# yz-cnsdqz/PSI-release

Measured on AMD Instinct MI355X. Metric: fitting iters/sec (SMPL-X+SDF+Chamfer), PROX-E batch=32, higher is better.
Workload: dtype f32

## Files before the change

### include/psi_hip.h

```cpp
#ifndef PSI_HIP_H
#define PSI_HIP_H

#include <stdint.h>

#ifdef __cplusplus
extern "C" {
#endif

#define PSI_EINVAL (-22)
#define PSI_ETIMEOUT (-110)
#define PSI_ENOMEM (-12)

const char *psi_last_error(void);
int psi_version(void);
int psi_device_info(int *cu_count, int *wave_size, int *clock_khz, int *is_gfx950);

int psi_chamfer_arith_mode(void);
size_t psi_chamfer_workspace_bytes(int B, int n, int m);
int psi_chamfer_forward(const float *xyz1, const float *xyz2, int B, int n, int m,
                        float *dist1, int32_t *idx1, float *dist2, int32_t *idx2,
                        void *workspace, void *stream);
int psi_scratch_release(void *stream, int all);
int psi_chamfer_backward(const float *xyz1, const float *xyz2, float *gradxyz1, float *gradxyz2,
                         const float *graddist1, const float *graddist2,
                         const int32_t *idx1, const int32_t *idx2, int B, int n, int m, void *stream);

typedef struct psi_nn_index psi_nn_index;
int psi_nn_index_create(psi_nn_index **out, const float *h_points, int m);
void psi_nn_index_destroy(psi_nn_index *index);
int psi_nn_index_query(const psi_nn_index *index, const float *xyz1, int B, int n, float *dist1, int32_t *idx1,
                       int32_t *hint, void *stream);

typedef struct psi_nn_index_set psi_nn_index_set;
int psi_nn_index_set_create(psi_nn_index_set **out, const psi_nn_index *const *indices, int S);
void psi_nn_index_set_destroy(psi_nn_index_set *set);
int psi_nn_index_set_query(const psi_nn_index_set *set, const int32_t *slot, const float *xyz1, int B, int n,
                           float *dist1, int32_t *idx1, void *stream);

int psi_sdf_sample_forward(const float *sdf, const int32_t *scene_id, const float *gmin, const float *gmax,
                           const float *verts, int B, int V, int D, int S, int align_corners,
                           float *out_sdf, float *out_grad, void *stream);
int psi_sdf_sample_backward(const float *grad_sdf, const float *out_grad, int B, int V,
                            float *grad_verts, void *stream);
int psi_sdf_penetration_stats(const float *sdf_vals, long n, float *stats, void *stream);

typedef struct psi_lbs_model psi_lbs_model;
int psi_lbs_create(psi_lbs_model **out, const float *h_v_template, const float *h_shapedirs,
                   const float *h_posedirs, const float *h_J_regressor, const float *h_weights,
                   const int32_t *h_parents, int V, int J, int NB);
void psi_lbs_destroy(psi_lbs_model *model);
size_t psi_lbs_workspace_floats(const psi_lbs_model *model, int B);
int psi_lbs_forward(const psi_lbs_model *model, const float *betas, const float *pose, const float *transl,
                    const float *cam_ext, int B, float *verts, float *joints, float *ws, void *stream);
int psi_lbs_backward(const psi_lbs_model *model, const float *grad_verts, const float *betas, const float *pose,
                     const float *cam_ext, int B, float *ws, float *grad_betas, float *grad_pose,
                     float *grad_transl, void *stream);

typedef struct psi_fit_engine psi_fit_engine;
typedef struct psi_fit_config {
    int B, n_contact, m_scene, D, align_corners, world_size, num_pca_comps, max_history;
    int nn_mode;
    float w_rec, w_vposer, w_contact, w_collision, contact_const;
    float lr, beta1, beta2, eps;
    int independent_bodies;
    int concurrent_engines;
    double lr_d, beta1_d, beta2_d;
} psi_fit_config;
int psi_fit_create(psi_fit_engine **out, const psi_lbs_model *lbs, const psi_fit_config *cfg,
                   const float *h_w1, const float *h_b1, const float *h_w2, const float *h_b2,
                   const float *h_w3, const float *h_b3, const float *h_lh_comp, const float *h_rh_comp,
                   const float *h_pose_mean, const int32_t *h_contact_ids,
                   const float *d_scene_verts, const float *d_sdf, const float *h_gmin, const float *h_gmax);
void psi_fit_destroy(psi_fit_engine *engine);
typedef struct psi_fit_scene {
    const float *d_verts;
    const float *d_sdf;
    int m, D;
    float gmin[3], gmax[3];
} psi_fit_scene;
int psi_fit_create_scenes(psi_fit_engine **out, const psi_lbs_model *lbs, const psi_fit_config *cfg,
                          const float *h_w1, const float *h_b1, const float *h_w2, const float *h_b2,
                          const float *h_w3, const float *h_b3, const float *h_lh_comp, const float *h_rh_comp,
                          const float *h_pose_mean, const int32_t *h_contact_ids,
                          const psi_fit_scene *h_scenes, int S);
int psi_fit_set_scene_slots(psi_fit_engine *engine, const int32_t *d_slot, void *stream);
int psi_fit_scene_count(const psi_fit_engine *engine);
int psi_fit_set_problem(psi_fit_engine *engine, const float *d_xhr, const float *d_x_init, const float *d_cam_ext,
                        int reset_optimizer, void *stream);
int psi_fit_forward(psi_fit_engine *engine, float *d_stats, int use_graph, void *stream);
int psi_fit_backward_step(psi_fit_engine *engine, const float *d_stats, int use_graph, void *stream);
int psi_fit_iterate(psi_fit_engine *engine, int n_iter, int use_graph, void *stream);
int psi_fit_read(psi_fit_engine *engine, float *d_x_out, float *d_history_out, int n_hist, int *h_step, void *stream);
int psi_fit_read_losses(psi_fit_engine *engine, int adam_step, float *d_out4, void *stream);
int psi_fit_decode_forward(psi_fit_engine *engine, const float *d_x75, const float *d_cam_ext, float *d_verts, void *stream);
int psi_fit_decode_backward(psi_fit_engine *engine, const float *d_grad_verts, float *d_grad_x75, void *stream);

#define PSI_DP_ID_BYTES 128
typedef struct psi_dp_comm psi_dp_comm;
int psi_dp_unique_id(char *h_id128);
int psi_dp_comm_create(psi_dp_comm **out, const char *h_id128, int rank, int world);
void psi_dp_comm_destroy(psi_dp_comm *comm);
int psi_dp_comm_info(const psi_dp_comm *comm, int *rank, int *world, int *rccl_version);
int psi_dp_allreduce_sum(psi_dp_comm *comm, float *d_buf, int n, void *stream);
int psi_fit_iterate_dp(psi_fit_engine *engine, psi_dp_comm *comm, int n_iter, int use_graph, float *d_stats, void *stream);
int psi_fit_dp_mode(const psi_fit_engine *engine);
int psi_stream_wait(void *stream, int timeout_ms);

int psi_fit_profile(psi_fit_engine *engine, int n_rep, char *h_names, int name_stride, float *h_ms, int max_stages,
                    int *h_n_stages, void *stream);
int psi_fit_copy_buffer(psi_fit_engine *engine, const char *name, float *d_out, long n_floats, void *stream);

size_t psi_linear_workspace_floats(int M, int N, int K);
int psi_linear_forward(const void *x, int x_is_bf16, const float *W, const float *bias, const float *residual, int M, int N, int K,
                       int act, float slope, float *y, float *act_out, float *ws, void *stream);
int psi_linear_forward3(const void *x, int x_is_bf16, const float *W, const float *bias, const float *residual, int M, int N, int K,
                        int act, float slope, float *y, float *act_out, float *ws, void *stream);
size_t psi_linear_backward_workspace_floats(int M, int N, int K);
int psi_linear_backward3(const float *gy, const float *act_out, const float *x, const float *W, int M, int N, int K, float slope, float *gx,
                         float *gW, float *gbias, float *ws, void *stream);
int psi_linear_backward(const float *gy, const float *act_out, const void *x, int x_is_bf16, const float *W, int M, int N, int K,
                        float slope, void *gx, float *gW, float *gbias, float *ws, void *stream);

size_t psi_bn_workspace_floats(long M, int C);
int psi_bn_forward(const void *x, const void *residual, const float *gamma, const float *beta, float *running_mean,
                   float *running_var, long long *num_batches_tracked, long M, int C, int relu, float momentum, float eps,
                   void *y, float *save_mean, float *save_invstd, float *ws, void *stream);
int psi_bn_backward(const void *dy, const void *x, const void *y, const float *gamma, const float *save_mean,
                    const float *save_invstd, long M, int C, int relu, void *dx, void *dresidual, float *dgamma, float *dbeta,
                    float *ws, void *stream);

int psi_conv3x3_supported(int Cin, int Cout, int H, int W);
int psi_conv3x3_forward(const void *x, const void *w, const float *bias, int N, int H, int W, int Cin, int Cout, void *y, void *stream);
size_t psi_conv3x3_wrw_workspace_floats(int N, int H, int W, int Cin, int Cout);
int psi_conv3x3_weight_grad(const void *x, const void *dy, int N, int H, int W, int Cin, int Cout, float *gw, float *ws, void *stream);
int psi_conv3x3_rotate_weight(const void *w, int Cin, int Cout, void *wt, void *stream);
int psi_conv3x3_prepare_weight(const float *w32, int Cin, int Cout, void *wb, void *wt, void *stream);

int psi_maxpool3x3s2_forward(const void *x, int N, int H, int W, int C, void *y, void *idx, void *stream);
int psi_maxpool3x3s2_backward(const void *dy, const void *idx, int N, int H, int W, int C, void *dx, void *stream);

int psi_conv2d_supported(int Cin, int Cout, int KH, int KW, int stride, int pad);
int psi_conv2d_forward(const void *x, int x_bf16, const float *w, const float *bias, int N, int H, int W, int Cin, int Cout, int KH, int KW,
                       int stride, int pad, void *y, int y_bf16, int nterm, void *stream);
int psi_conv2d_input_grad(const void *dy, int dy_bf16, const float *wt, int N, int H, int W, int Cin, int Cout, int KH, int KW, int stride, int pad,
                          void *dx, int dx_bf16, int nterm, void *stream);
int psi_conv2d_prepared_ok(int Cin, int Cout, int KH, int KW, int stride, int pad);
int psi_conv2d_prepare_weight(const float *w, int Cout, int KH, int KW, int Cin, int nterm, void *wf, void *wt, void *stream);
int psi_conv2d_forward_p(const void *x, int x_bf16, const void *wf, const float *bias, int N, int H, int W, int Cin, int Cout, int KH, int KW,
                         int stride, int pad, void *y, int y_bf16, int nterm, void *stream);
int psi_conv2d_input_grad_p(const void *dy, int dy_bf16, const void *wt, int N, int H, int W, int Cin, int Cout, int KH, int KW, int stride, int pad,
                            void *dx, int dx_bf16, int nterm, void *stream);
size_t psi_conv2d_wgrad_workspace_floats(int N, int H, int W, int Cin, int Cout, int KH, int KW, int stride, int pad);
int psi_conv2d_weight_grad(const void *x, int x_bf16, const void *dy, int dy_bf16, int N, int H, int W, int Cin, int Cout, int KH, int KW, int stride,
                           int pad, float *gw, float *ws, int nterm, void *stream);
int psi_adam_step(void *const *p, const void *const *g, void *const *m, void *const *v, const long *n, int count, float *step, unsigned *ticket,
                  double lr, double beta1, double beta2, double eps, double weight_decay, void *stream);
int psi_bn_forward_t(const void *x, int map_f32, const void *residual, const float *gamma, const float *beta, float *running_mean,
                     float *running_var, long long *num_batches_tracked, long M, int C, int relu, float momentum, float eps, void *y,
                     float *save_mean, float *save_invstd, float *ws, int eval_mode, void *stream);
int psi_bn_backward_t(const void *dy, int map_f32, const void *x, const void *y, const float *gamma, const float *beta, const float *save_mean,
                      const float *save_invstd, long M, int C, int relu, void *dx, void *dresidual, float *dgamma, float *dbeta, float *ws,
                      void *stream);
int psi_maxpool3x3s2_forward_t(const void *x, int map_f32, int N, int H, int W, int C, void *y, void *idx, void *stream);
int psi_maxpool3x3s2_backward_t(const void *dy, int map_f32, const void *idx, int N, int H, int W, int C, void *dx, void *stream);

size_t psi_cvae_losses_workspace_floats(void);
int psi_cvae_target(const float *xh72, const float *cam_int, const float *max_d, int B, float *out75, void *stream);
int psi_cvae_losses_forward(const float *rec75, const float *target75, const float *xh72, const float *cam_int, const float *max_d,
                            const float *mu0, const float *logvar0, int nz0, const float *mu1, const float *logvar1, int nz1, int B,
                            float w_rec, float w_kl, float w_vposer, float fca, const float *fca_dev, float *ws, float *xh_rec75,
                            float *losses5, void *stream);
int psi_cvae_losses_backward(const float *rec75, const float *target75, const float *xh72, const float *cam_int, const float *max_d,
                             const float *mu0, const float *logvar0, int nz0, const float *mu1, const float *logvar1, int nz1, int B,
                             float w_rec, float w_kl, float w_vposer, float fca, const float *fca_dev, const float *xh_rec75,
                             const float *g_losses5, const float *g_xh_rec75, float *g_rec75, float *g_mu0, float *g_logvar0,
                             float *g_mu1, float *g_logvar1, void *stream);

size_t psi_scene_losses_workspace_floats(void);
int psi_scene_losses_forward(const float *dist, long n_contact, const float *sdf_vals, long n_sdf, float w_contact, float w_collision,
                             float gate, float *ws, float *losses2, float *stats2, void *stream);
int psi_scene_losses_backward(const float *g_losses2, const float *stats2, const float *dist, const float *xyz1, const int32_t *idx,
                              const int32_t *slot, const float *verts_table, long m, const int32_t *vid, const float *sdf_vals,
                              const float *sdf_grad, int B, int V, int n_c, float w_contact, float w_collision, float gate,
                              const int32_t *chain, float *g_verts, void *stream);
int psi_contact_slot_chain(const int32_t *vid, int n_c, int32_t *chain, void *stream);

int psi_lbs_sdf_counts(const psi_lbs_model *model, const float *betas, const float *pose, const float *transl,
                       const float *cam_ext, int B, const float *sdf, const int32_t *scene_id, const float *gmin,
// ... 133 lines not shown
```

### psi-release_amd/csrc/fit.hip

```cpp
#include "psi_internal.h"
#ifdef PSI_HEAD_STOPS
__device__ int psi_dbg_sstop;
#define PSI_SSTOP(k) do { if (psi_dbg_sstop == (k)) return; } while (0)
__device__ int psi_dbg_pstop;
#define PSI_PSTOP(k) do { if (psi_dbg_pstop == (k)) asm volatile("s_endpgm"); } while (0)
#define PSI_TRACE(lo, hi) PsiBlockTrace trace_((lo), (hi))
__device__ unsigned long long psi_dbg_tl[4 * 8192];
struct PsiBlockTrace {
    unsigned long long t0;
    int kind;
    int sel_lo, sel_hi;
    __device__ PsiBlockTrace(int lo = 9, int hi = 10) : t0(wall_clock64()), kind(0), sel_lo(lo), sel_hi(hi) {}
    __device__ ~PsiBlockTrace()
    {
        const unsigned bid = blockIdx.y * gridDim.x + blockIdx.x;
        if (psi_dbg_sstop < sel_lo || psi_dbg_sstop > sel_hi || threadIdx.x != 0 || bid >= 8192) return;
        unsigned long long *o = psi_dbg_tl + 4 * (size_t)bid;
        o[0] = t0;
        o[1] = wall_clock64();
        o[2] = (unsigned long long)__builtin_amdgcn_s_getreg((31 << 11) | 4) | ((unsigned long long)__builtin_amdgcn_s_getreg((31 << 11) | 20) << 32);
        o[3] = (unsigned long long)kind;
    }
};
extern "C" int psi_dbg_timeline(unsigned long long *out, int nblocks)
{
    return (int)hipMemcpyFromSymbol(out, HIP_SYMBOL(psi_dbg_tl), sizeof(unsigned long long) * 4 * (size_t)(nblocks < 8192 ? nblocks : 8192));
}
#endif
#include "lbs_device.h"
#include "lbs_joint_device.h"
#include "sdf_device.h"
#include "nnindex_device.h"
#include <initializer_list>
#include <limits.h>
#include <memory>
#include <math.h>
#include <stdlib.h>
#include <string.h>
#include <type_traits>
#include <vector>

namespace {

constexpr int NH = 512;
constexpr int NZ = 32;
constexpr int NJ6 = 126;
constexpr int XD = 75;
#ifndef PSI_HEAD_THREADS
#define PSI_HEAD_THREADS 512
#endif
constexpr int HB = PSI_HEAD_THREADS;
static_assert(HB >= 384 && HB % 128 == 0, "the head / tail kernels place work on threads up to 256 + 75");
constexpr int KQ = HB / 128;
constexpr int KS3 = HB / 32;
constexpr int OS1 = HB / 8;
typedef float f4 __attribute__((ext_vector_type(4)));

struct FitDev {
    int B, V, Vpad, J, NB, n_c, m, D, align_corners, world, ncomp, nfp, nsdfblk;
    int indep;
    float w_rec, w_vp, w_contact, w_col, cconst;
    float lr, beta1, beta2, eps;
    float one_m_beta1, one_m_beta2;
    double lr_d, beta1_d, beta2_d;
    const float *W1T, *b1, *W2T, *b2, *W3T, *b3;
    const float *W1, *W2, *W3;
    const float *lhc, *rhc, *pose_mean;
    const int *vid;
    const int *cs_ptr, *cs_idx;
    const int *cs_first;
    const float *scene, *sdf, *gmin, *gmax;
    const float *sdf_cells;
    const float *Wct;
    float *x, *xhr, *cam, *adam_m, *adam_v;
    int *step;
    float *h1, *h2, *o6, *betas20, *pose, *transl, *verts, *og, *gq, *fpart, *penpart, *recpart, *vppart;
    float *cverts;
    float *g_betas, *g_pose, *g_transl, *g_rot;
    unsigned long long *hx_o6, *hx_gh1;
    unsigned *hx_epoch;
    int *hx_err;
    int hc;
#ifdef PSI_HEAD_STOPS
    int stop_h, stop_t;
#define HSTOP(k) do { if (f.stop_h == (k)) return; } while (0)
#define TSTOP(k) do { if (f.stop_t == (k)) return; } while (0)
#else
#define HSTOP(k)
#define TSTOP(k)
#endif
    int *nn_hint;
    float *history;
    int max_hist;
    int fused_bwd, ncp, ncp3;
    float *glc, *gvpc, *vpc;
    float *gtc_part;
#ifndef PSI_GV_SLOTS
#define PSI_GV_SLOTS 1024
#endif
    static_assert(PSI_GV_SLOTS >= 128, "one slot per body and class at least: fused_bwd runs batches up to 128 (merged_scene)");
    unsigned *gvbits;
    int gv_sps;
    const float *dirs_ch;
    const float *WTt_c;
    float *gA_part, *gfeat_part;
    float *spb;
    int nsv, nsv_c, nsn_m, nsn_c, spm, spc;
    unsigned long long *penmask;
    int pen_skip;
};

__device__ __forceinline__ float leaky(float v, float slope) { return v > 0.0f ? v : v * slope; }
// ... 49 lines not shown
    if (m22 < 1e-6f) {
        if (m00 > m11) {
            t = 1 + m00 - m11 - m22;
            q[0] = m12 - m21; q[1] = t; q[2] = m01 + m10; q[3] = m20 + m02;
        } else {
            t = 1 - m00 + m11 - m22;
            q[0] = m20 - m02; q[1] = m01 + m10; q[2] = t; q[3] = m12 + m21;
        }
    } else {
        if (m00 < -m11) {
            t = 1 - m00 - m11 + m22;
            q[0] = m01 - m10; q[1] = m20 + m02; q[2] = m12 + m21; q[3] = t;
        } else {
            t = 1 + m00 + m11 + m22;
            q[0] = t; q[1] = m12 - m21; q[2] = m20 - m02; q[3] = m01 - m10;
        }
    }
    float sc = sqrtf(t);
    for (int i = 0; i < 4; i++) q[i] = q[i] / sc * 0.5f;
    float s2 = q[1] * q[1] + q[2] * q[2] + q[3] * q[3];
    float s = sqrtf(s2);
    float two_theta = 2.0f * (q[0] < 0.0f ? atan2f(-s, -q[0]) : atan2f(s, q[0]));
    float k = s2 > 0.0f ? two_theta / s : 2.0f;
    aa[0] = q[1] * k; aa[1] = q[2] * k; aa[2] = q[3] * k;
}

__device__ __forceinline__ float block_sum(float v, float *sh)
{
#pragma unroll
    for (int o = 32; o > 0; o >>= 1) v += __shfl_down(v, o, 64);
    __syncthreads();
    if ((threadIdx.x & 63) == 0) sh[threadIdx.x >> 6] = v;
    __syncthreads();
    float s = 0;
    for (int i = 0; i < (int)(blockDim.x >> 6); i++) s += sh[i];
    return s;
}

__device__ __forceinline__ void block_sum2(float &a, float &c, float *sh2)
{
#pragma unroll
    for (int o = 32; o > 0; o >>= 1) {
        a += __shfl_down(a, o, 64);
        c += __shfl_down(c, o, 64);
    }
    __syncthreads();
    if ((threadIdx.x & 63) == 0) {
        sh2[2 * (threadIdx.x >> 6)] = a;
        sh2[2 * (threadIdx.x >> 6) + 1] = c;
    }
    __syncthreads();
    float sa = 0, sc = 0;
    for (int i = 0; i < (int)(blockDim.x >> 6); i++) {
        sa += sh2[2 * i];
        sc += sh2[2 * i + 1];
    }
    a = sa;
    c = sc;
}

__device__ __forceinline__ void hx_put(unsigned long long *p, float v, unsigned tag)
{
    __hip_atomic_store(p, ((unsigned long long)tag << 32) | (unsigned long long)__float_as_uint(v), __ATOMIC_RELAXED, __HIP_MEMORY_SCOPE_AGENT);
}
__device__ __forceinline__ unsigned long long hx_peek(unsigned long long *p)
{
    return __hip_atomic_load(p, __ATOMIC_RELAXED, __HIP_MEMORY_SCOPE_AGENT);
}
constexpr int HX_MAX_POLLS = 1 << 20;
__device__ __forceinline__ float hx_value(unsigned long long *p, unsigned long long w, unsigned tag, int *err)
{
    int polls = 0;
    while ((unsigned)(w >> 32) != tag) {
        if (++polls > HX_MAX_POLLS) {
            *err = 1;
            break;
        }
        __builtin_amdgcn_s_sleep(1);
        w = hx_peek(p);
    }
    return __uint_as_float((unsigned)w);
}

template <int C>
__global__ __launch_bounds__(HB) void head_fwd_kernel(FitDev f, PsiLbsView lv)
{
    constexpr int NS = NH / C;
    constexpr int NQ = NS / 4;
    constexpr int KSPL = HB / NQ;
    constexpr int KPER = NH / KSPL;
    constexpr int KPER3 = NS / KS3;
    constexpr int K1 = NZ / KQ;
    constexpr int PRE2 = C > 1 ? 16 : 0;
    constexpr int PRE3 = C > 1 ? (KPER3 < 4 ? KPER3 : 4) : 0;
    static_assert(KPER % 16 == 0 && KPER3 >= 1 && NS >= 64, "cluster too wide for the thread layout");
    const int b = blockIdx.x / C, c = blockIdx.x % C, t = threadIdx.x;
    const bool last = c == C - 1;
    __shared__ float sx[XD + 5], sh1[NH], sh2[NS], so6[128], red[HB / 64], spose[PSI_JP * 3], sbetas[32], sJ[PSI_JP][3];
    __shared__ f4 part4[HB], part3[KS3][32];
    const int og1 = t & 127, kq1 = t >> 7, og2 = t % NQ, ks2 = t / NQ, og3 = t & 31, ks3 = t >> 5;
    const float *w1 = f.W1T + (size_t)(kq1 * K1) * NH + og1 * 4;
    const float *w2 = f.W2T + (size_t)(ks2 * KPER) * NH + c * NS + og2 * 4;
    const float *w3 = f.W3T + (size_t)(c * NS + ks3 * KPER3) * 128 + og3 * 4;
    f4 w1p[K1], w2p[PRE2 ? PRE2 : 1], w3p[PRE3 ? PRE3 : 1];
#pragma unroll
    for (int k = 0; k < K1; k++) w1p[k] = *(const f4 *)(w1 + (size_t)k * NH);
#pragma unroll
    for (int k = 0; k < PRE2; k++) w2p[k] = *(const f4 *)(w2 + (size_t)k * NH);
#pragma unroll
    for (int k = 0; k < PRE3; k++) w3p[k] = *(const f4 *)(w3 + (size_t)k * 128);
    const float *x = f.x + (size_t)b * XD;
    if (t < XD) sx[t] = x[t];
    if (t >= 64 && t < 96) sbetas[t - 64] = t - 64 < 10 ? x[9 + (t - 64)] : 0.0f;
    unsigned tag = 0;
    float pm[3] = {0, 0, 0}, b3v = 0.0f;
    PsiJump jp;
    for (int r = 0; r < PSI_NJUMP; r++) jp.a[r] = -1;
    if (C > 1) tag = f.hx_epoch[b] + 1u;
    f4 b1v = {0, 0, 0, 0};
    if (t < 128) b1v = *(const f4 *)(f.b1 + t * 4);
    const float b2v = t < NS ? f.b2[c * NS + t] : 0.0f;
    if (last) {
        if (t < 22)
            for (int e = 0; e < 3; e++) pm[e] = f.pose_mean[t * 3 + e];
        if (t < 128) b3v = f.b3[t];
        jp = psi_load_jump(lv.m);
    }
    __syncthreads();
    HSTOP(1);
    if (c == 0) {
        float dr = t < XD ? fabsf(f.xhr[(size_t)b * XD + t] - sx[t]) : 0.0f;
        float sr = block_sum(dr, red);
        float dz = t < NZ ? sx[19 + t] * sx[19 + t] : 0.0f;
        float sz = block_sum(dz, red);
        if (t == 0) {
            f.recpart[b] = sr;
            f.vppart[b] = sz;
        }
    }
    if (last) {
        if (t >= 64 && t < 64 + 9) {
            int e = 66 + (t - 64);
            spose[e] = f.pose_mean[e];
        } else if (t >= 128 && t < 128 + 90) {
            int e = t - 128;
            const float *comp = e < 45 ? f.lhc : f.rhc;
            const float *hx = sx + (e < 45 ? 51 : 63);
            int cc = e < 45 ? e : e - 45;
            float a = 0;
            for (int i = 0; i < f.ncomp; i++) a += hx[i] * comp[i * 45 + cc];
            spose[75 + e] = a + f.pose_mean[75 + e];
        }
        psi_pose_fwd_rest(lv.m, sbetas, sJ);
    }
    HSTOP(2);
    const float *z = sx + 19;
    {
        f4 a = {0, 0, 0, 0};
#pragma unroll
        for (int k = 0; k < K1; k++) a += w1p[k] * z[kq1 * K1 + k];
        part4[kq1 * 128 + og1] = a;
    }
    __syncthreads();
    if (t < 128) {
        f4 a = b1v;
#pragma unroll
        for (int q = 0; q < KQ; q++) a += part4[q * 128 + t];
        for (int e = 0; e < 4; e++) sh1[t * 4 + e] = leaky(a[e], 0.2f);
    }
    __syncthreads();
    HSTOP(3);
    {
        f4 a0 = {0, 0, 0, 0}, a1 = {0, 0, 0, 0};
        const float *h = sh1 + ks2 * KPER;
#pragma unroll
        for (int k = 0; k < PRE2; k += 2) {
            a0 += w2p[k] * h[k];
            a1 += w2p[k + 1] * h[k + 1];
        }
#pragma unroll 8
        for (int k = PRE2; k < KPER; k += 2) {
            a0 += *(const f4 *)(w2 + (size_t)k * NH) * h[k];
            a1 += *(const f4 *)(w2 + (size_t)(k + 1) * NH) * h[k + 1];
        }
        part4[ks2 * NQ + og2] = a0 + a1;
    }
    __syncthreads();
    if (t < NS) {
        float a = b2v;
        const float *p = (const float *)part4;
#pragma unroll
        for (int q = 0; q < KSPL; q++) a += p[q * NS + t];
        a = leaky(a, 0.2f);
        sh2[t] = a;
        f.h2[(size_t)b * NH + c * NS + t] = a;
    }
    if (c == 0)
        for (int o = t; o < NH; o += HB) f.h1[(size_t)b * NH + o] = sh1[o];
    __syncthreads();
    HSTOP(4);
    {
        f4 a = {0, 0, 0, 0};
        const float *h = sh2 + ks3 * KPER3;
#pragma unroll
        for (int k = 0; k < PRE3; k++) a += w3p[k] * h[k];
#pragma unroll
        for (int k = PRE3; k < KPER3; k++) a += *(const f4 *)(w3 + (size_t)k * 128) * h[k];
        part3[ks3][og3] = a;
    }
    __syncthreads();
    HSTOP(5);
    if (t < 128) {
        float a = 0.0f;
        const float *p = (const float *)part3;
#pragma unroll
        for (int ks = 0; ks < KS3; ks++) a += p[ks * 128 + t];
        if (C == 1) {
            so6[t] = a + b3v;
        } else if (!last) {
            hx_put(f.hx_o6 + ((size_t)b * C + c) * 128 + t, a, tag);
        } else {
            unsigned long long *p8 = f.hx_o6 + (size_t)b * C * 128 + t;
            unsigned long long w[C - 1 ? C - 1 : 1];
#pragma unroll
            for (int cc = 0; cc < C - 1; cc++) w[cc] = hx_peek(p8 + cc * 128);
            float o = b3v;
#pragma unroll
            for (int cc = 0; cc < C - 1; cc++) o += hx_value(p8 + cc * 128, w[cc], tag, f.hx_err);
            so6[t] = o + a;
        }
    }
    if (C > 1 && !last) return;
    __syncthreads();
    HSTOP(6);
    if (t < NJ6) f.o6[(size_t)b * 128 + t] = so6[t];
    if (t < 22) {
        float R[9], aa[3];
        gs_forward(t == 0 ? sx + 3 : so6 + (t - 1) * 6, R);
        rotmat_to_aa(R, aa);
        for (int e = 0; e < 3; e++) spose[t * 3 + e] = aa[e] + pm[e];
    }
    __syncthreads();
    HSTOP(7);
    psi_pose_fwd_chain(lv.m, spose, nullptr, f.B, b, sJ, jp, lv.feat, lv.R, lv.G, lv.A, nullptr);
    HSTOP(8);
    psi_pose_fwd_rest_store(lv.m, sbetas, f.B, b, sJ, lv.feat, lv.Jl);
    for (int i = t; i < f.J * 3; i += HB) f.pose[(size_t)b * f.J * 3 + i] = spose[i];
    if (t < f.NB) f.betas20[(size_t)b * f.NB + t] = sbetas[t];
    if (t >= 64 && t < 67) f.transl[(size_t)b * 3 + (t - 64)] = sx[t - 64];
    if (C > 1 && t == 0) f.hx_epoch[b] = tag;
}

struct SdfPenEpilogue {
    PsiSdfGrid G;
    const float *sdf, *gmin, *gmax;
    float *og, *penpart;
    int D, align_corners, Vpad;
    const int *contact_of;
    float s[2];
    bool neg[2];
    float *cverts;
    const int *cs_ptr, *cs_idx;
    int n_c;
    float *gl, *gvp, *gtp;
    int Npad, B;
    float gm[2][3], gs[2][3];
    float gvmax[2];
    unsigned *gmaxp;
    int gv_sps;
    unsigned long long *penmask;
    __device__ __forceinline__ void store(float *verts, size_t body_off, int b, int v, unsigned v12, float x, float y, float z) const
    {
        if (!contact_of) {
            if (verts) psi_st(verts + body_off, v12, psi_p3{x, y, z});
            return;
        }
        const int cw = psi_ld<int>(contact_of, (unsigned)v * 4u);
        if (!(cw >> 24)) return;
        float *row = cverts + (size_t)b * n_c * 3;
        psi_st(row, (unsigned)(cw & 0xffffff) * 12u, psi_p3{x, y, z});
        if ((cw >> 24) > 1)
            for (int ci = cs_ptr[v] + 1; ci < cs_ptr[v + 1]; ci++) psi_st(row, (unsigned)cs_idx[ci] * 12u, psi_p3{x, y, z});
    }
    __device__ __forceinline__ void vertex(int n, int b, int v, float x, float y, float z, bool live) { vertex_at(G, n, b, v, x, y, z, live); }
    __device__ __forceinline__ void vertex_at(const PsiSdfGrid &G, int n, int b, int v, float x, float y, float z, bool live)
    {
        s[n] = 0.0f;
        neg[n] = false;
#pragma unroll
        for (int a = 0; a < 3; a++) gm[n][a] = 0.0f;
        if (!live) return;
        float g[3];
        if (G.cells) {
            bool in[3];
            const float val = psi_sdf_sample_cells(G, x, y, z, g, in);
            neg[n] = val < 0.0f;
#pragma unroll
            for (int a = 0; a < 3; a++) g[a] = (neg[n] && in[a]) ? g[a] : 0.0f;
            s[n] = neg[n] ? -val : 0.0f;
        } else {
            const float val = psi_trilinear(sdf, gmin, gmax, x, y, z, D, align_corners, g);
            neg[n] = val < 0.0f;
#pragma unroll
            for (int a = 0; a < 3; a++) g[a] = neg[n] ? g[a] : 0.0f;
            s[n] = neg[n] ? -val : 0.0f;
        }
        if (gl) {
#pragma unroll
            for (int a = 0; a < 3; a++) gm[n][a] = g[a];
            return;
        }
        psi_st(og + (size_t)b * Vpad * 4, (unsigned)v * 16u, f4{g[0], g[1], g[2], 0.0f});
    }
    __device__ __forceinline__ void backward(int n, int b, unsigned v12, const psi_f2 (&T2)[6], const float *C)
    {
        if (!gl) return;
        const float gx = gm[n][0], gy = gm[n][1], gz = gm[n][2];
        float lx = gx, ly = gy, lz = gz;
        if (C) {
            lx = psi_dot3(C[0], C[4], C[8], gx, gy, gz);
            ly = psi_dot3(C[1], C[5], C[9], gx, gy, gz);
            lz = psi_dot3(C[2], C[6], C[10], gx, gy, gz);
        }
        psi_st(gl + (size_t)b * Npad, v12, psi_p3{lx, ly, lz});
        const float vx = psi_dot3(T2[0].x, T2[2].x, T2[4].x, lx, ly, lz), vy = psi_dot3(T2[0].y, T2[2].y, T2[4].y, lx, ly, lz),
                    vz = psi_dot3(T2[1].x, T2[3].x, T2[5].x, lx, ly, lz);
        psi_st(gvp + (size_t)b * Npad, v12, psi_p3{vx, vy, vz});
// ... 867 lines not shown
            for (int cc = 0; cc < C - 1; cc++) o += hx_value(p8 + (size_t)cc * NH, w[cc], tag, f.hx_err);
            sga1[t] = (o + a) * (h1v > 0.0f ? 1.0f : 0.2f);
        }
    }
    __syncthreads();
    TSTOP(6);
    {
        f4 a = {0, 0, 0, 0};
        if (C == 1) {
#pragma unroll
            for (int i = 0; i < O1; i++) a += *(const f4 *)(w1 + (size_t)i * NZ) * sga1[os1 * O1 + i];
        } else {
#pragma unroll
            for (int i = 0; i < O1; i++) a += w1p[i] * sga1[os1 * O1 + i];
        }
        part1[os1][kg1] = a;
    }
    __syncthreads();
    if (t < 8) {
        f4 a = {0, 0, 0, 0};
        for (int os = 0; os < OS1; os++) a += part1[os][t];
        for (int e = 0; e < 4; e++) sgx[19 + t * 4 + e] = a[e];
    }
    __syncthreads();
    TSTOP(7);
    if (C > 1 && t == 0) f.hx_epoch[f.B + b] = tag;
    if (!ADAM) {
        if (t < XD) g_out[(size_t)b * XD + t] = sgx[t];
        return;
    }
    if (ta >= 0 && ta < XD) {
        const float Bg = f.indep ? 1.0f : (float)f.B * (float)f.world;
        float g = sgx[ta];
        float df = xhrv - sx[ta];
        g += f.w_rec / (Bg * XD) * (df > 0.0f ? -1.0f : (df < 0.0f ? 1.0f : 0.0f));
        if (ta >= 19 && ta < 19 + NZ) g += f.w_vp / (Bg * NZ) * 2.0f * sx[ta];
        size_t o = (size_t)b * XD + ta;
        float m = am * f.beta1 + f.one_m_beta1 * g;
        float v = av * f.beta2 + f.one_m_beta2 * g * g;
        f.adam_m[o] = m;
        f.adam_v[o] = v;
        float denom = sqrtf(v) / bc2_sqrt + f.eps;
        f.x[o] = sx[ta] - step_size * (m / denom);
    }
}

__global__ void sdf_to_cells_kernel(const float *__restrict__ src, float *__restrict__ dst, int D)
{
    const int nbr = D >> 2;
    const size_t i = (size_t)blockIdx.x * 256 + threadIdx.x, n = (size_t)D * D * D * 8;
    if (i >= n) return;
    const int c = (int)(i & 7), l = (int)((i >> 3) & 63);
    const size_t br = i >> 9;
    const int bz = (int)(br % nbr), by = (int)((br / nbr) % nbr), bx = (int)(br / ((size_t)nbr * nbr));
    const int ix = min(4 * bx + (l >> 4) + (c >> 2), D - 1), iy = min(4 * by + ((l >> 2) & 3) + ((c >> 1) & 1), D - 1),
              iz = min(4 * bz + (l & 3) + (c & 1), D - 1);
    dst[i] = src[((size_t)ix * D + iy) * D + iz];
}

__global__ void scene_slots_kernel(const int *__restrict__ src, int *__restrict__ dst, int B, int S)
{
    const int b = blockIdx.x * 256 + threadIdx.x;
    if (b < B) dst[b] = min(max(src[b], 0), S - 1);
}

__global__ void adam_reset_kernel(float *m, float *v, int *step, int n)
{
    int i = blockIdx.x * 256 + threadIdx.x;
    if (i < n) { m[i] = 0.0f; v[i] = 0.0f; }
    if (i == 0) *step = 0;
}

}

#ifndef PSI_FIT_SEARCH_LANES_DEFAULT
#define PSI_FIT_SEARCH_LANES_DEFAULT 2
#endif
#ifndef PSI_GRAPH_UNROLL
#define PSI_GRAPH_UNROLL 10
#endif
constexpr int GRAPH_UNROLL = PSI_GRAPH_UNROLL;

struct FitKnobs {
    bool split_scene, keep_verts, no_fused_bwd, sdf_linear, scene_skin_first, bwdv_mb, no_pen_skip, bwd_pf1;
    int head_cluster, skin_nb, ska_nbody, search_lanes;
#ifdef PSI_HEAD_STOPS
    int head_stop, tail_stop, skin_stop;
#endif
};

static FitKnobs fit_read_knobs()
{
    auto is = [](const char *name, char c) { const char *v = getenv(name); return v && v[0] == c; };
    auto num = [](const char *name) { const char *v = getenv(name); return v ? atoi(v) : 0; };
    FitKnobs k = {};
    k.split_scene = is("PSI_SPLIT_SCENE", '1');
    k.keep_verts = is("PSI_KEEP_VERTS", '1');
    k.no_fused_bwd = is("PSI_FIT_FUSED_BWD", '0');
    k.no_pen_skip = is("PSI_FIT_PEN_SKIP", '0');
    k.bwd_pf1 = is("PSI_FIT_BWD_PF", '1');
    k.sdf_linear = is("PSI_SDF_LINEAR", '1');
    k.scene_skin_first = is("PSI_SCENE_ORDER", '1');
    k.bwdv_mb = is("PSI_BWDV_MB", '1');
    const int hc = num("PSI_HEAD_CLUSTER");
    if (hc == 1 || hc == 2 || hc == 4 || hc == 8) k.head_cluster = hc;
    if (getenv("PSI_SKIN_NB")) k.skin_nb = num("PSI_SKIN_NB") == 2 ? 2 : 1;
    k.ska_nbody = psi_ska_nbody_override(SKA_NBODY);
    const int sl = num("PSI_FIT_SEARCH_LANES");
    if (sl == 2 || sl == 4) k.search_lanes = sl;
#ifdef PSI_HEAD_STOPS
    k.head_stop = num("PSI_HEAD_STOP");
    k.tail_stop = num("PSI_TAIL_STOP");
    k.skin_stop = num("PSI_SKIN_STOP");
#endif
    return k;
}

struct FitModes {
    bool self_skin;
    bool merged_scene;
    bool keep_verts;
    bool fused_bwd;
    int skin_nb;
    int search_lanes;
    int hc;
    int gv_sps;
    PsiStreamSplit split;
};

static FitModes fit_decide(const psi_fit_config *cfg, const FitKnobs &knobs, int J, int ncp3, const PsiLbsCounts &mc)
{
    FitModes d = {};
    d.self_skin = cfg->nn_mode == 1 && J <= PSI_JP - 8 && psikd::kd_qpb(psikd::LPQ_OPS) == psikd::kd_qpb(2);
    d.search_lanes = knobs.search_lanes ? knobs.search_lanes : mc.compressed_weights ? 4 : PSI_FIT_SEARCH_LANES_DEFAULT;
    d.merged_scene = d.self_skin && cfg->B <= 128 && !knobs.split_scene;
    d.keep_verts = !d.merged_scene || knobs.keep_verts;
    const long bodies = (long)cfg->B * (cfg->concurrent_engines > 1 ? cfg->concurrent_engines : 1);
    d.hc = bodies <= 32 ? 8 : bodies <= 64 ? 4 : bodies <= 128 ? 2 : 1;
    if (knobs.head_cluster) d.hc = knobs.head_cluster;
    d.gv_sps = 16;
    while (d.gv_sps > 1 && (long)d.gv_sps * cfg->B > PSI_GV_SLOTS) d.gv_sps >>= 1;
    d.split = psi_stream_split(mc.Npad / 16, ncp3 / 16, mc.nsn);
    d.fused_bwd = d.merged_scene && !knobs.no_fused_bwd && d.split.nsn_c > 0;
    d.skin_nb = cfg->B > 128 && !mc.compressed_weights ? 2 : 1;
    if (knobs.skin_nb) d.skin_nb = knobs.skin_nb;
    return d;
}

struct FitBuf {
    void *field;
    size_t off, bytes;
    const void *src;
    int fill;
    const char *name;
};
struct FitBlob {
    std::vector<FitBuf> bufs;
    size_t size;
    size_t zero_begin;
    template <class T>
    void add(T *&field, size_t bytes, const void *src, int fill, const char *name)
    {
        bufs.push_back({&field, size, bytes, src, fill, name});
        size += (bytes + 255) & ~(size_t)255;
    }
    template <class T> void upload(T *&field, const void *src, size_t bytes) { add(field, bytes, src, 0, nullptr); }
    template <class T> void zero(T *&field, size_t bytes, const char *name = nullptr) { add(field, bytes, nullptr, 0, name); }
    template <class T> void ones(T *&field, size_t bytes, const char *name = nullptr) { add(field, bytes, nullptr, 0xff, name); }
};

struct FitPlan {
    int mt;
    int kgroups, n_blend;
    PsiSkaPlan ska;
    bool pf1;
};
static FitPlan fit_plan_make(const FitDev &f, const LbsDev &m, int ska_nbody_override, bool pf1)
{
    FitPlan p;
    p.kgroups = m.Kpad / 64;
    p.mt = f.B > 32 ? 4 : (f.B > 16 ? 2 : 1);
    p.n_blend = p.kgroups * (f.nsn_m + f.nsn_c) * psi_cdiv(f.B, 16 * p.mt);
    p.ska = psi_ska_plan(f.B, f.nsv, f.nsv_c, SKA_NBODY, ska_nbody_override);
    p.pf1 = pf1;
    return p;
}

struct FitGraph { hipGraph_t g; hipGraphExec_t exec; bool ready; };

struct FitCaptured {
    enum Kind { Ok, Refused, Error } kind;
    int rc;
};

template <class Seq>
static FitCaptured fit_graph_capture(FitGraph *G, hipStream_t st, Seq &&seq)
{
    auto failed = [](const char *what, hipError_t he) {
        psi_set_error("%s failed: %s", what, hipGetErrorString(he));
        return FitCaptured{FitCaptured::Error, (int)he};
    };
    if (!st) {
        psi_set_error("invalid argument: graph capture needs a non-default stream");
        return {FitCaptured::Error, PSI_EINVAL};
    }
    hipError_t he = hipStreamBeginCapture(st, hipStreamCaptureModeRelaxed);
    if (he != hipSuccess) return failed("begin of the stream capture", he);
    const int rc = seq();
    hipGraph_t g = nullptr;
    he = hipStreamEndCapture(st, &g);
    if (!rc && he == hipSuccess) {
        he = hipGraphInstantiate(&G->exec, g, nullptr, nullptr, 0);
        if (he != hipSuccess) {
            (void)hipGraphDestroy(g);
            return failed("hipGraphInstantiate", he);
        }
        G->g = g;
        G->ready = true;
        return {FitCaptured::Ok, 0};
    }
    if (g) (void)hipGraphDestroy(g);
    if (!rc) (void)failed("hipStreamEndCapture", he);
    const bool refused = (he >= hipErrorStreamCaptureUnsupported && he <= hipErrorStreamCaptureWrongThread) || rc == 1000 + 4 || rc == 1000 + 5;
    return {refused ? FitCaptured::Refused : FitCaptured::Error, rc ? rc : (int)he};
}

static int fit_graph_launch(const FitGraph &G, hipStream_t st)
{
    PSI_CHECK_HIP(hipGraphLaunch(G.exec, st));
    return 0;
}

static void fit_graph_drop(FitGraph *G)
{
    if (G->ready) {
        (void)hipGraphExecDestroy(G->exec);
        (void)hipGraphDestroy(G->g);
    }
    *G = FitGraph{};
}

struct FitGraphTier { int iters; FitGraph *graph; };

template <class Seq>
static FitCaptured fit_run_graphs(hipStream_t st, int n_iter, int *done, std::initializer_list<FitGraphTier> tiers, Seq &&one)
{
    for (const FitGraphTier &t : tiers) {
        if (n_iter - *done < t.iters) continue;
        if (!t.graph->ready) {
            const FitCaptured c = fit_graph_capture(t.graph, st, [&]() {
                int rc = 0;
                for (int i = 0; i < t.iters && !rc; i++) rc = one();
                return rc;
            });
            if (c.kind != FitCaptured::Ok) return c;
        }
        for (; *done + t.iters <= n_iter; *done += t.iters)
            if (int rc = fit_graph_launch(*t.graph, st)) return {FitCaptured::Error, rc};
    }
    return {FitCaptured::Ok, 0};
}

enum {
    FIT_G_ITER_1, FIT_G_ITER_N, FIT_G_ITER_2N,
    FIT_G_HALF_FWD, FIT_G_HALF_BWD,
    FIT_G_DP_1, FIT_G_DP_N,
    FIT_N_GRAPHS
};

struct psi_fit_engine {
    FitDev d;
    PsiSdfGrid grid;
    const psi_lbs_model *lbs;
    psi_nn_index *nn_index;
    float *lbs_ws;
    PsiLbsView lv;
    void *nn_ws;
    char *blob;
    FitBlob table;
    float *stats_local;
    FitKnobs knobs;
    FitModes mode;
    FitPlan plan;
    int n_scenes;
    psi_nn_index **scene_index;
    float **scene_vol;
    psikd::KdDev *d_kd_tab;
    PsiSdfGrid *d_grid_tab;
    int *d_slot;
    int kd_rows;
    FitGraph graphs[FIT_N_GRAPHS];
    const float *half_stats[2];
    const void *dp_comm;
    const float *dp_stats;
    bool dp_warm;
    bool dp_no_graph;
};

static void launch_head_fwd(const FitDev &f, const PsiLbsView &lv, hipStream_t st)
{
    const dim3 g(f.B * f.hc), blk(HB);
    switch (f.hc) {
    case 8: hipLaunchKernelGGL(head_fwd_kernel<8>, g, blk, 0, st, f, lv); break;
    case 4: hipLaunchKernelGGL(head_fwd_kernel<4>, g, blk, 0, st, f, lv); break;
    case 2: hipLaunchKernelGGL(head_fwd_kernel<2>, g, blk, 0, st, f, lv); break;
    default: hipLaunchKernelGGL(head_fwd_kernel<1>, g, blk, 0, st, f, lv); break;
    }
}

template <bool ADAM>
static void launch_head_bwd(const FitDev &f, const PsiLbsView &lv, float *g_out, hipStream_t st)
{
    const dim3 g(f.B * f.hc), blk(HB);
    switch (f.hc) {
    case 8: hipLaunchKernelGGL((head_bwd_adam_kernel<8, ADAM>), g, blk, 0, st, f, lv, g_out); break;
    case 4: hipLaunchKernelGGL((head_bwd_adam_kernel<4, ADAM>), g, blk, 0, st, f, lv, g_out); break;
    case 2: hipLaunchKernelGGL((head_bwd_adam_kernel<2, ADAM>), g, blk, 0, st, f, lv, g_out); break;
    default: hipLaunchKernelGGL((head_bwd_adam_kernel<1, ADAM>), g, blk, 0, st, f, lv, g_out); break;
    }
}

enum class FitStats {
    Finalize,
    Backward,
    Caller
};

static inline FitStats fit_stats_source(const psi_fit_engine *e, FitStats wish)
{
    return wish == FitStats::Backward && !e->mode.fused_bwd && e->d.B >= PSI_SKIN_MB_MIN_B ? FitStats::Finalize : wish;
}

static int fit_launch_stats(psi_fit_engine *e, float *stats, hipStream_t st)
{
    hipLaunchKernelGGL(loss_finalize_kernel, dim3(1), dim3(1024), 0, st, e->d, stats);
    PSI_CHECK_LAUNCH("loss_finalize_kernel");
    psi_mark("loss_finalize_kernel", st);
    return 0;
}

template <int NB, bool SCENES, int LPQ>
static void launch_fwd_scene(const psi_fit_engine *e, float gscale, hipStream_t st)
{
    const FitDev &f = e->d;
    const int nqb = f.nfp, n_kd = nqb * f.B, skin_first = e->knobs.scene_skin_first ? 1 : 0;
    const dim3 grid(n_kd + f.nsdfblk * psi_cdiv(f.B, NB));
    FitDev fk = f;
    if (!e->mode.keep_verts) fk.verts = nullptr;
    const auto epi = make_sdf_epilogue<SCENES>(f, e->grid, false, e->mode.fused_bwd ? &e->lv : nullptr, e->d_grid_tab, e->d_slot);
    SceneTrees<SCENES> T;
    int rows;
    if constexpr (SCENES) {
        T = e->d_kd_tab;
        rows = e->kd_rows;
    } else {
        T = psi_nn_index_dev(e->nn_index);
        rows = T.rows;
    }
    hipLaunchKernelGGL((fwd_scene_kernel<NB, SCENES, LPQ>), grid, dim3(256), psikd::kd_lds_bytes(LPQ, rows), st, fk, e->lv.m, e->lv.A, e->lv.v_posed, T, n_kd, nqb, rows,
                       gscale, skin_first, epi);
}

template <int NB, bool SCENES>
static void launch_skin_fwd_sdf(const psi_fit_engine *e, bool all_verts, hipStream_t st)
{
    const FitDev &f = e->d;
    hipLaunchKernelGGL((skin_fwd_sdf_kernel<NB, SCENES>), dim3(f.nsdfblk, psi_cdiv(f.B, NB)), dim3(PSI_SKIN_BLK), 0, st, e->lv.m, e->lv.A, e->lv.v_posed,
                       f.transl, f.cam, f.B, f.verts, make_sdf_epilogue<SCENES>(f, e->grid, !all_verts, nullptr, e->d_grid_tab, e->d_slot));
}

template <class L>
static void fit_scene_dispatch(const psi_fit_engine *e, L &&launch)
{
    using One = std::integral_constant<int, 1>;
    using Two = std::integral_constant<int, 2>;
    switch ((e->n_scenes ? 2 : 0) | (e->mode.skin_nb == 2 ? 1 : 0)) {
    case 0: launch(One{}, std::false_type{}); break;
    case 1: launch(Two{}, std::false_type{}); break;
    case 2: launch(One{}, std::true_type{}); break;
    default: launch(Two{}, std::true_type{}); break;
    }
}

static int fit_forward(psi_fit_engine *e, float *stats, hipStream_t st, FitStats who)
{
    FitDev &f = e->d;
    launch_head_fwd(f, e->lv, st);
    PSI_CHECK_LAUNCH("head_fwd_kernel");
    psi_mark("head_fwd_kernel", st);
    int rc = psi_lbs_blend_forward(e->lbs, f.B, e->lbs_ws, st);
    if (rc) return rc;
    float gscale = f.w_contact / ((f.indep ? 1.0f : (float)f.B * (float)f.world) * (float)f.n_c);
    if (e->nn_index && e->mode.merged_scene) {
        fit_scene_dispatch(e, [&](auto nb, auto scenes) {
            if (e->mode.search_lanes == 2) launch_fwd_scene<decltype(nb)::value, decltype(scenes)::value, 2>(e, gscale, st);
            else launch_fwd_scene<decltype(nb)::value, decltype(scenes)::value, 4>(e, gscale, st);
        });
        PSI_CHECK_LAUNCH("fwd_scene_kernel");
        psi_mark("fwd_scene_kernel", st);
    } else {
        const bool all_verts = !e->nn_index || e->knobs.keep_verts;
        fit_scene_dispatch(e, [&](auto nb, auto scenes) { launch_skin_fwd_sdf<decltype(nb)::value, decltype(scenes)::value>(e, all_verts, st); });
        PSI_CHECK_LAUNCH("skin_fwd_sdf_kernel");
        psi_mark("skin_fwd_sdf_kernel", st);
        if (e->n_scenes)
            rc = psi_nn_index_contact_set(e->d_kd_tab, e->d_slot, e->kd_rows, all_verts ? f.verts : f.cverts, all_verts ? (long)f.V * 3 : (long)f.n_c * 3,
                                          all_verts ? f.vid : nullptr, f.B, f.n_c, f.cconst, gscale, f.gq, f.fpart, f.nn_hint, st);
        else if (e->nn_index && !all_verts)
            rc = psi_nn_index_contact(e->nn_index, f.cverts, (long)f.n_c * 3, nullptr, f.B, f.n_c, f.cconst, gscale, f.gq, f.fpart, f.nn_hint, st);
        else if (e->nn_index)
            rc = psi_nn_index_contact(e->nn_index, f.verts, (long)f.V * 3, f.vid, f.B, f.n_c, f.cconst, gscale, f.gq, f.fpart, f.nn_hint, st);
        else
            rc = psi_nn_contact(f.verts, (long)f.V * 3, f.vid, f.scene, f.B, f.n_c, f.m, e->nn_ws, f.cconst, gscale, f.gq, f.fpart, nullptr, st);
        if (rc) return rc;
    }
    return fit_stats_source(e, who) == FitStats::Finalize ? fit_launch_stats(e, stats, st) : 0;
}

static int fit_backward_joint(psi_fit_engine *e, float *stats, hipStream_t st, FitStats who)
{
    FitDev &f = e->d;
    const FitPlan &p = e->plan;
    const dim3 grid(p.ska.n_ska + p.n_blend + (fit_stats_source(e, who) == FitStats::Backward ? 1 : 0));
#define PSI_LAUNCH_FIT_JOINT(MT_, PFM_, PFC_)                                                                                      \
    hipLaunchKernelGGL((fit_bwd_joint_kernel<MT_, PFM_, PFC_>), grid, dim3(256), 0, st, f, e->lv.m, e->lv.g_vp, e->lv.gl, e->lv.v_posed, p.ska, p.n_blend, p.kgroups, stats)
#define PSI_LAUNCH_FIT_JOINT_MT(MT_)                                                                                               \
    do {                                                                                                                           \
        if (p.pf1) PSI_LAUNCH_FIT_JOINT(MT_, 1, 1);                                                                                \
        else PSI_LAUNCH_FIT_JOINT(MT_, PSI_FIT_PF_MODEL, PSI_FIT_PF_CONTACT);                                                      \
    } while (0)
    if (p.mt == 4) PSI_LAUNCH_FIT_JOINT_MT(4);
    else if (p.mt == 2) PSI_LAUNCH_FIT_JOINT_MT(2);
    else PSI_LAUNCH_FIT_JOINT_MT(1);
#undef PSI_LAUNCH_FIT_JOINT_MT
#undef PSI_LAUNCH_FIT_JOINT
    PSI_CHECK_LAUNCH("fit_bwd_joint_kernel");
    psi_mark("bwd_joint_kernel", st);
    return 0;
}

static int fit_backward_tail(psi_fit_engine *e, float *stats, hipStream_t st)
{
    FitDev &f = e->d;
    const long nred = (long)f.B * PSI_JP * 16 + (long)f.B * e->lv.m.Kpad + (long)f.B * 4;
    hipLaunchKernelGGL(fit_reduce_kernel, dim3(psi_cdiv(nred * PSI_RSPL, 256)), dim3(256), 0, st, f, e->lv, stats);
    PSI_CHECK_LAUNCH("fit_reduce_kernel");
    psi_mark("reduce_partials_kernel", st);
    launch_head_bwd<true>(f, e->lv, nullptr, st);
    PSI_CHECK_LAUNCH("head_bwd_adam_kernel");
    psi_mark("head_bwd_adam_kernel", st);
    return 0;
}

static int fit_backward(psi_fit_engine *e, float *stats, hipStream_t st, FitStats who)
{
    FitDev &f = e->d;
    if (e->mode.fused_bwd) {
        int rc = fit_backward_joint(e, stats, st, who);
        return rc ? rc : fit_backward_tail(e, stats, st);
    }
    const bool big = f.B >= PSI_SKIN_MB_MIN_B;
    const bool mb = big && (e->lv.m.Wc || e->knobs.bwdv_mb);
    const dim3 bgrid(f.nsdfblk, mb ? psi_cdiv(f.B, PSI_SKIN_MB) : f.B);
#define PSI_LAUNCH_BWD_V(...)                                                                                                      \
    hipLaunchKernelGGL((psi_skin_bwd_v_kernel<__VA_ARGS__>), bgrid, dim3(PSI_SKIN_BLK), 0, st, e->lv.m, e->lv.A, src, f.cam, f.B, e->lv.gl, e->lv.g_vp, e->lv.gt_part_w)
    if (fit_stats_source(e, who) == FitStats::Backward) {
        const FitGradSource<true> src{f, stats, 0.0f, nullptr, 0, {}, false};
        if (mb) psi_launch_skin_bwd_v_mb(e->lv.m, e->lv.A, src, f.cam, f.B, e->lv.gl, e->lv.g_vp, e->lv.gt_part_w, st);
        else PSI_LAUNCH_BWD_V(FitGradSource<true>);
    } else {
        const FitGradSource<false> src{f, stats, 0.0f, nullptr, 0, {}, false};
        if (mb) psi_launch_skin_bwd_v_mb(e->lv.m, e->lv.A, src, f.cam, f.B, e->lv.gl, e->lv.g_vp, e->lv.gt_part_w, st);
        else if (big) PSI_LAUNCH_BWD_V(FitGradSource<false>, PsiBlendPipelined);
        else PSI_LAUNCH_BWD_V(FitGradSource<false>);
    }
#undef PSI_LAUNCH_BWD_V
    PSI_CHECK_LAUNCH("skin_bwd_v_grad_kernel");
    psi_mark("skin_bwd_v_grad_kernel", st);
    int rc = psi_lbs_backward_joint_parts(e->lbs, f.B, e->lbs_ws, f.g_transl, st);
    if (rc) return rc;
    launch_head_bwd<true>(f, e->lv, nullptr, st);
    PSI_CHECK_LAUNCH("head_bwd_adam_kernel");
    psi_mark("head_bwd_adam_kernel", st);
    return 0;
}

static int fit_build_scenes(psi_fit_engine *e, const psi_fit_scene *h_scenes, int S);

static inline size_t fit_x_bytes(const FitDev &f) { return (size_t)f.B * XD * 4; }
static inline size_t fit_cam_bytes(const FitDev &f) { return (size_t)f.B * 16 * 4; }
static inline size_t fit_hint_bytes(const FitDev &f) { return (size_t)f.B * f.n_c * 4; }
static inline hipError_t fit_hints_reset(const FitDev &f, hipStream_t st) { return hipMemsetAsync(f.nn_hint, 0xff, fit_hint_bytes(f), st); }

static inline size_t sdf_cells_bytes(int D) { return (size_t)D * D * D * 32; }
static void sdf_cells_fill(const float *d_sdf, float *d_cells, int D)
{
    hipLaunchKernelGGL(sdf_to_cells_kernel, dim3((unsigned)psi_cdiv((long)(sdf_cells_bytes(D) / 4), 256)), dim3(256), 0, 0, d_sdf, d_cells, D);
}

static int fit_scene_index(psi_nn_index **out, const float *d_verts, int m, hipError_t *err)
{
    std::vector<float> hs((size_t)m * 3);
    *err = hipMemcpy(hs.data(), d_verts, hs.size() * 4, hipMemcpyDeviceToHost);
    return *err == hipSuccess ? psi_nn_index_create(out, hs.data(), m) : (int)*err;
}

static int fit_create(psi_fit_engine **out, const psi_lbs_model *lbs, const psi_fit_config *cfg,
                      const float *h_w1, const float *h_b1, const float *h_w2, const float *h_b2,
                      const float *h_w3, const float *h_b3, const float *h_lh_comp, const float *h_rh_comp,
                      const float *h_pose_mean, const int32_t *h_contact_ids,
                      const float *d_scene_verts, const float *d_sdf, const float *h_gmin, const float *h_gmax,
                      const psi_fit_scene *h_scenes, int S)
{
    PSI_REQUIRE(out && lbs && cfg && h_w1 && h_b1 && h_w2 && h_b2 && h_w3 && h_b3 && h_lh_comp && h_rh_comp && h_pose_mean &&
                h_contact_ids && d_scene_verts && d_sdf && h_gmin && h_gmax, "null pointer");
    int V, J, NB;
    psi_lbs_dims(lbs, &V, &J, &NB);
    PSI_REQUIRE(J == 55 && NB >= 10 && NB <= 32, "the fused engine is SMPL-X shaped (J=55, 10..32 betas)");
    PSI_REQUIRE(cfg->B > 0 && cfg->n_contact > 0 && cfg->n_contact < (1 << 24) && cfg->m_scene > 0 && cfg->D >= 2 && cfg->world_size >= 1, "bad sizes");
    PSI_REQUIRE(cfg->num_pca_comps > 0 && cfg->num_pca_comps <= 12, "1..12 hand PCA components");
    PSI_REQUIRE(!(cfg->independent_bodies && cfg->world_size > 1), "independent bodies have no cross-rank coupling: use world_size 1");
    for (int i = 0; i < 66; i++) PSI_REQUIRE(h_pose_mean[i] == 0.0f, "pose_mean must be zero for global_orient/body joints");
    for (int i = 0; i < cfg->n_contact; i++) PSI_REQUIRE(h_contact_ids[i] >= 0 && h_contact_ids[i] < V, "contact id out of range");
    PsiLbsCounts mc;
    if (int rcv = psi_lbs_counts(lbs, cfg->B, &mc)) return rcv;
    psi_fit_engine *e = new psi_fit_engine();
    std::unique_ptr<psi_fit_engine, void (*)(psi_fit_engine *)> owner(e, psi_fit_destroy);
    const FitKnobs &knobs = e->knobs = fit_read_knobs();
    e->lbs = lbs;
    FitDev &f = e->d;
    f.B = cfg->B; f.V = V; f.J = J; f.NB = NB; f.n_c = cfg->n_contact; f.m = cfg->m_scene; f.D = cfg->D;
    f.align_corners = cfg->align_corners; f.world = cfg->world_size; f.ncomp = cfg->num_pca_comps;
    f.indep = cfg->independent_bodies ? 1 : 0;
    f.w_rec = cfg->w_rec; f.w_vp = cfg->w_vposer; f.w_contact = cfg->w_contact; f.w_col = cfg->w_collision; f.cconst = cfg->contact_const;
    f.lr = cfg->lr; f.beta1 = cfg->beta1; f.beta2 = cfg->beta2; f.eps = cfg->eps;
    f.lr_d = cfg->lr_d != 0.0 ? cfg->lr_d : (double)cfg->lr;
    f.beta1_d = cfg->beta1_d != 0.0 ? cfg->beta1_d : (double)cfg->beta1;
    f.beta2_d = cfg->beta2_d != 0.0 ? cfg->beta2_d : (double)cfg->beta2;
    f.one_m_beta1 = (float)(1.0 - f.beta1_d);
    f.one_m_beta2 = (float)(1.0 - f.beta2_d);
    f.nsdfblk = psi_cdiv(V, 256);
    f.Vpad = f.nsdfblk * 256;
    f.nfp = cfg->nn_mode == 1 ? psi_nn_index_fparts(f.n_c) : psi_nn_contact_fparts(f.n_c);
    f.max_hist = cfg->max_history > 0 ? cfg->max_history : 1024;
    f.ncp = psi_cdiv(f.n_c, 256) * 256;
    f.ncp3 = 3 * f.ncp;
    f.nsv = mc.nsv;
    f.nsv_c = f.ncp / 256;
    f.scene = d_scene_verts;
    f.sdf = d_sdf;
    const FitModes &mode = e->mode = fit_decide(cfg, knobs, J, f.ncp3, mc);
    f.hc = mode.hc;
    f.gv_sps = mode.gv_sps;
    f.fused_bwd = mode.fused_bwd ? 1 : 0;
    f.pen_skip = mode.fused_bwd && !knobs.no_pen_skip ? 1 : 0;
    f.nsn_m = mode.split.nsn_m; f.nsn_c = mode.split.nsn_c; f.spm = mode.split.spm; f.spc = mode.split.spc;
#ifdef PSI_HEAD_STOPS
    f.stop_h = knobs.head_stop;
    f.stop_t = knobs.tail_stop;
    (void)hipMemcpyToSymbol(HIP_SYMBOL(psi_dbg_sstop), &knobs.skin_stop, sizeof(int));
    (void)hipMemcpyToSymbol(HIP_SYMBOL(psi_dbg_pstop), &f.stop_t, sizeof(int));
#endif
    const size_t B = (size_t)f.B;
    std::vector<float> W1T((size_t)NZ * NH), W2T((size_t)NH * NH), W3T((size_t)NH * 128, 0.0f), b3p(128, 0.0f);
    memcpy(b3p.data(), h_b3, NJ6 * 4);
    for (int o = 0; o < NH; o++) for (int k = 0; k < NZ; k++) W1T[(size_t)k * NH + o] = h_w1[(size_t)o * NZ + k];
    for (int o = 0; o < NH; o++) for (int k = 0; k < NH; k++) W2T[(size_t)k * NH + o] = h_w2[(size_t)o * NH + k];
    for (int o = 0; o < NJ6; o++) for (int k = 0; k < NH; k++) W3T[(size_t)k * 128 + o] = h_w3[(size_t)o * NH + k];
    std::vector<int> cs_ptr(V + 1, 0), cs_idx(f.n_c), cs_first(V, 0);
    for (int i = 0; i < f.n_c; i++) cs_ptr[h_contact_ids[i] + 1]++;
    for (int v = 0; v < V; v++) cs_ptr[v + 1] += cs_ptr[v];
    {
        std::vector<int> fill(cs_ptr.begin(), cs_ptr.end() - 1);
        for (int i = 0; i < f.n_c; i++) cs_idx[fill[h_contact_ids[i]]++] = i;
        for (int v = 0; v < V; v++)
            if (cs_ptr[v + 1] > cs_ptr[v]) cs_first[v] = cs_idx[cs_ptr[v]] | (std::min(cs_ptr[v + 1] - cs_ptr[v], 127) << 24);
    }
    const size_t hand_pca = (size_t)f.ncomp * 45 * 4, hidden = B * NH * 4, betas = B * NB * 4, pose = B * J * 3 * 4, transl = B * 3 * 4,
                 crows = B * f.n_c * 3 * 4, per_body = B * 4, slot_rows = B * f.ncp3 * 4;
    FitBlob &T = e->table;
    T.upload(f.W1T, W1T.data(), W1T.size() * 4);
    T.upload(f.b1, h_b1, NH * 4);
    T.upload(f.W2T, W2T.data(), W2T.size() * 4);
    T.upload(f.b2, h_b2, NH * 4);
    T.upload(f.W3T, W3T.data(), W3T.size() * 4);
    T.upload(f.b3, b3p.data(), 128 * 4);
    T.upload(f.W1, h_w1, (size_t)NH * NZ * 4);
    T.upload(f.W2, h_w2, (size_t)NH * NH * 4);
    T.upload(f.W3, h_w3, (size_t)NJ6 * NH * 4);
    T.upload(f.lhc, h_lh_comp, hand_pca);
    T.upload(f.rhc, h_rh_comp, hand_pca);
    T.upload(f.pose_mean, h_pose_mean, (size_t)J * 3 * 4);
    T.upload(f.vid, h_contact_ids, (size_t)f.n_c * sizeof(int32_t));
    T.upload(f.cs_ptr, cs_ptr.data(), cs_ptr.size() * sizeof(int));
    T.upload(f.cs_idx, cs_idx.data(), cs_idx.size() * sizeof(int));
    T.upload(f.cs_first, cs_first.data(), cs_first.size() * sizeof(int));
    T.upload(f.gmin, h_gmin, 12);
    T.upload(f.gmax, h_gmax, 12);
    T.zero_begin = T.size;
    T.zero(f.x, fit_x_bytes(f));
    T.zero(f.xhr, fit_x_bytes(f));
    T.zero(f.cam, fit_cam_bytes(f));
    T.zero(f.adam_m, fit_x_bytes(f), "adam_m");
    T.zero(f.adam_v, fit_x_bytes(f), "adam_v");
    T.zero(f.step, 256);
    T.zero(f.h1, hidden);
    T.zero(f.h2, hidden);
    T.zero(f.o6, B * 128 * 4);
    T.zero(f.betas20, betas);
    T.zero(f.pose, pose, "pose");
    T.zero(f.transl, transl);
    T.zero(f.verts, B * V * 3 * 4, "verts");
    T.zero(f.cverts, crows);
    T.zero(f.og, B * f.Vpad * 4 * 4);
    T.zero(f.gq, crows);
    T.zero(f.fpart, B * f.nfp * 4, "fpart");
    T.zero(f.penpart, B * f.nsdfblk * 2 * 4);
    T.zero(f.recpart, per_body);
    T.zero(f.vppart, per_body);
    T.zero(f.g_betas, betas);
    T.zero(f.g_pose, pose, "g_pose");
    T.zero(f.g_transl, transl, "g_transl");
    T.zero(f.g_rot, B * J * 9 * 4, "g_rot");
    T.zero(f.history, (size_t)f.max_hist * 4 * 4);
    T.zero(e->stats_local, 256);
    T.ones(f.nn_hint, fit_hint_bytes(f), "nn_hint");
    T.zero(f.hx_o6, B * f.hc * 128 * 8);
    T.zero(f.hx_gh1, B * f.hc * NH * 8);
    T.zero(f.hx_epoch, 2 * B * 4);
    T.zero(f.Wct, (size_t)f.n_c * PSI_JP * 4);
    if (mode.fused_bwd) {
        T.zero(f.glc, slot_rows, "glc");
        T.zero(f.gvpc, slot_rows, "gvpc");
        T.zero(f.vpc, slot_rows, "vpc");
        T.zero(f.gtc_part, B * f.nfp * 4 * 4, "gtc_part");
        T.zero(f.gvbits, 2 * PSI_GV_SLOTS * 4);
        T.zero(f.WTt_c, (size_t)f.ncp * PSI_JP * 4);
        T.zero(f.dirs_ch, (size_t)f.ncp3 * mc.Kpad * 4);
        T.zero(f.gA_part, (size_t)(f.nsv + f.nsv_c) * B * PSI_JP * 16 * 4);
        T.zero(f.gfeat_part, (size_t)(f.nsn_m + f.nsn_c) * B * mc.Kpad * 4);
        T.zero(f.spb, per_body, "spb");
        T.zero(f.penmask, B * (f.Vpad / 64) * 8, "penmask");
    }
    const bool cells = !h_scenes && psi_sdf_cells_fit(f.D) && !knobs.sdf_linear;
// ... 203 lines not shown
    if (!use_graph) return half();
    FitGraph *G = &e->graphs[FIT_G_HALF_FWD + which];
    if (G->ready && e->half_stats[which] != stats) fit_graph_drop(G);
    if (!G->ready) {
        const FitCaptured c = fit_graph_capture(G, st, half);
        if (c.kind != FitCaptured::Ok) return c.rc;
        e->half_stats[which] = stats;
    }
    return fit_graph_launch(*G, st);
}

extern "C" int psi_fit_forward(psi_fit_engine *e, float *d_stats, int use_graph, void *stream)
{
    PSI_REQUIRE(e, "null engine");
    return fit_half(e, 0, d_stats ? d_stats : e->stats_local, use_graph, (hipStream_t)stream);
}

extern "C" int psi_fit_backward_step(psi_fit_engine *e, const float *d_stats, int use_graph, void *stream)
{
    PSI_REQUIRE(e, "null engine");
    return fit_half(e, 1, (float *)(d_stats ? d_stats : e->stats_local), use_graph, (hipStream_t)stream);
}

extern "C" int psi_fit_iterate(psi_fit_engine *e, int n_iter, int use_graph, void *stream)
{
    PSI_REQUIRE(e && n_iter >= 0, "bad arguments");
    PSI_REQUIRE(e->d.world == 1, "psi_fit_iterate is the single-process path; data-parallel runs call forward / all-reduce / backward_step");
    hipStream_t st = (hipStream_t)stream;
    auto one = [&]() { return fit_iteration(e, st); };
    int done = 0, rc = 0;
    if (!use_graph) {
        for (; done < n_iter && !rc; done++) rc = one();
        return rc;
    }
    return fit_run_graphs(st, n_iter, &done,
                          {{2 * GRAPH_UNROLL, &e->graphs[FIT_G_ITER_2N]}, {GRAPH_UNROLL, &e->graphs[FIT_G_ITER_N]}, {1, &e->graphs[FIT_G_ITER_1]}}, one).rc;
}

extern "C" int psi_fit_iterate_dp(psi_fit_engine *e, psi_dp_comm *comm, int n_iter, int use_graph, float *d_stats, void *stream)
{
    PSI_REQUIRE(e && comm && n_iter >= 0, "bad arguments");
    PSI_REQUIRE(psi_dp_world(comm) == e->d.world, "the communicator's size differs from psi_fit_config.world_size");
    hipStream_t st = (hipStream_t)stream;
    float *stats = d_stats ? d_stats : e->stats_local;
    auto one = [&]() -> int {
        if (e->mode.fused_bwd) {
            int rc = fit_forward(e, stats, st, FitStats::Backward);
            if (!rc) rc = fit_backward_joint(e, stats, st, FitStats::Backward);
            if (!rc) rc = psi_dp_allreduce_sum(comm, stats, 6, st);
            return rc ? rc : fit_backward_tail(e, stats, st);
        }
        int rc = fit_forward(e, stats, st, FitStats::Finalize);
        if (!rc) rc = psi_dp_allreduce_sum(comm, stats, 6, st);
        if (!rc) rc = fit_backward(e, stats, st, FitStats::Finalize);
        return rc;
    };
    if (e->dp_comm != comm || e->dp_stats != stats) {
        fit_graph_drop(&e->graphs[FIT_G_DP_1]);
        fit_graph_drop(&e->graphs[FIT_G_DP_N]);
        e->dp_warm = e->dp_warm && e->dp_comm == comm;
        e->dp_comm = comm;
        e->dp_stats = stats;
    }
    int done = 0;
    auto eager = [&](int upto) {
        int rc = 0;
        for (; done < upto && !rc; done++) rc = one();
        return rc;
    };
    if (!use_graph || (!e->dp_warm && n_iter > 0)) {
        if (int rc = eager(use_graph ? 1 : n_iter)) return rc;
        e->dp_warm = true;
        if (!use_graph) return 0;
    }
    if (!e->dp_no_graph) {
        const FitCaptured c = fit_run_graphs(st, n_iter, &done, {{GRAPH_UNROLL, &e->graphs[FIT_G_DP_N]}, {1, &e->graphs[FIT_G_DP_1]}}, one);
        if (c.kind != FitCaptured::Refused) return c.rc;
        (void)hipGetLastError();
        e->dp_no_graph = true;
    }
    return eager(n_iter);
}

extern "C" int psi_fit_dp_mode(const psi_fit_engine *e)
{
    if (!e || !e->dp_warm) return 0;
    return e->dp_no_graph ? 2 : 1;
}

extern "C" int psi_fit_decode_forward(psi_fit_engine *e, const float *d_x75, const float *d_cam_ext, float *d_verts, void *stream)
{
    PSI_REQUIRE(e && d_x75 && d_cam_ext && d_verts, "null pointer");
    FitDev &f = e->d;
    hipStream_t st = (hipStream_t)stream;
    PSI_CHECK_HIP(hipMemcpyAsync(f.x, d_x75, fit_x_bytes(f), hipMemcpyDeviceToDevice, st));
    PSI_CHECK_HIP(hipMemcpyAsync(f.cam, d_cam_ext, fit_cam_bytes(f), hipMemcpyDeviceToDevice, st));
    launch_head_fwd(f, e->lv, st);
    PSI_CHECK_LAUNCH("head_fwd_kernel");
    int rc = psi_lbs_blend_forward(e->lbs, f.B, e->lbs_ws, st);
    if (rc) return rc;
    hipLaunchKernelGGL(psi_skin_fwd_kernel<PsiSkinNoEpilogue>, dim3(f.nsdfblk, f.B), dim3(PSI_SKIN_BLK), 0, st, e->lv.m, e->lv.A,
                       e->lv.v_posed, f.transl, f.cam, f.B, d_verts, PsiSkinNoEpilogue());
    PSI_CHECK_LAUNCH("skin_fwd_kernel");
    return 0;
}

extern "C" int psi_fit_decode_backward(psi_fit_engine *e, const float *d_grad_verts, float *d_grad_x75, void *stream)
{
    PSI_REQUIRE(e && d_grad_verts && d_grad_x75, "null pointer");
    FitDev &f = e->d;
    hipStream_t st = (hipStream_t)stream;
    if (f.B >= PSI_SKIN_MB_MIN_B)
        psi_launch_skin_bwd_v_mb(e->lv.m, e->lv.A, PsiGradFromMemory{d_grad_verts, f.V}, f.cam, f.B, e->lv.gl, e->lv.g_vp, e->lv.gt_part_w, st);
    else
        hipLaunchKernelGGL(psi_skin_bwd_v_kernel<PsiGradFromMemory>, dim3(f.nsdfblk, f.B), dim3(PSI_SKIN_BLK), 0, st, e->lv.m, e->lv.A,
                           PsiGradFromMemory{d_grad_verts, f.V}, f.cam, f.B, e->lv.gl, e->lv.g_vp, e->lv.gt_part_w);
    PSI_CHECK_LAUNCH("skin_bwd_v_kernel");
    int rc = psi_lbs_backward_joint_parts(e->lbs, f.B, e->lbs_ws, f.g_transl, st);
    if (rc) return rc;
    launch_head_bwd<false>(f, e->lv, d_grad_x75, st);
    PSI_CHECK_LAUNCH("head_bwd_kernel");
    return 0;
}

extern "C" int psi_fit_profile(psi_fit_engine *e, int n_rep, char *h_names, int name_stride, float *h_ms, int max_stages,
                               int *h_n_stages, void *stream)
{
    PSI_REQUIRE(e && h_names && h_ms && h_n_stages && n_rep > 0 && max_stages > 0 && name_stride >= 16, "bad arguments");
    PSI_REQUIRE(e->d.world == 1, "profile the single-process path");
    hipStream_t st = (hipStream_t)stream;
    PsiStageTimer tm;
    memset(&tm, 0, sizeof(tm));
    for (int i = 0; i < 48; i++) PSI_CHECK_HIP(hipEventCreate(&tm.ev[i]));
    std::vector<double> acc(48, 0.0);
    int n_st = 0, rc = 0;
    for (int r = 0; r < n_rep && !rc; r++) {
        tm.n = 0;
        (void)hipEventRecord(tm.ev[0], st);
        tm.name[0] = "start";
        tm.n = 1;
        g_psi_timer = &tm;
        rc = fit_iteration(e, st);
        g_psi_timer = nullptr;
        if (rc) break;
        PSI_CHECK_HIP(hipStreamSynchronize(st));
        n_st = tm.n - 1;
        for (int i = 1; i < tm.n; i++) {
            float ms = 0;
            (void)hipEventElapsedTime(&ms, tm.ev[i - 1], tm.ev[i]);
            acc[i - 1] += ms;
        }
    }
    for (int i = 0; i < 48; i++) (void)hipEventDestroy(tm.ev[i]);
    if (rc) return rc;
    if (n_st > max_stages) n_st = max_stages;
    for (int i = 0; i < n_st; i++) {
        h_ms[i] = (float)(acc[i] / n_rep);
        strncpy(h_names + (size_t)i * name_stride, tm.name[i + 1], name_stride - 1);
        h_names[(size_t)i * name_stride + name_stride - 1] = 0;
    }
    *h_n_stages = n_st;
    return 0;
}

extern "C" int psi_fit_read(psi_fit_engine *e, float *d_x_out, float *d_history_out, int n_hist, int *h_step, void *stream)
{
    PSI_REQUIRE(e, "null engine");
    FitDev &f = e->d;
    hipStream_t st = (hipStream_t)stream;
    if (d_x_out) PSI_CHECK_HIP(hipMemcpyAsync(d_x_out, f.x, fit_x_bytes(f), hipMemcpyDeviceToDevice, st));
    if (d_history_out && n_hist > 0) {
        if (n_hist > f.max_hist) n_hist = f.max_hist;
        PSI_CHECK_HIP(hipMemcpyAsync(d_history_out, f.history, (size_t)n_hist * 16, hipMemcpyDeviceToDevice, st));
    }
    if (h_step) {
        int hs[2] = {0, 0};
        PSI_CHECK_HIP(hipMemcpyAsync(hs, f.step, 8, hipMemcpyDeviceToHost, st));
        PSI_CHECK_HIP(hipStreamSynchronize(st));
        *h_step = hs[0];
        if (hs[1]) {
            (void)hipMemsetAsync(f.hx_err, 0, 4, st);
            psi_set_error("psi_fit_read: a head / tail cluster exchange timed out (a producer workgroup never published its partials); "
                          "the results of this fit are invalid.  PSI_HEAD_CLUSTER=1 runs the kernels without clusters");
            return 902;
        }
    }
    return 0;
}

extern "C" int psi_fit_read_losses(psi_fit_engine *e, int adam_step, float *d_out4, void *stream)
{
    PSI_REQUIRE(e && d_out4 && adam_step >= 1, "bad arguments");
    FitDev &f = e->d;
    PSI_CHECK_HIP(hipMemcpyAsync(d_out4, f.history + (size_t)((adam_step - 1) % f.max_hist) * 4, 16, hipMemcpyDeviceToDevice, (hipStream_t)stream));
    return 0;
}

extern "C" int psi_fit_copy_buffer(psi_fit_engine *e, const char *name, float *d_out, long n_floats, void *stream)
{
    PSI_REQUIRE(e && name && d_out && n_floats >= 0, "bad arguments");
    FitDev &f = e->d;
    const PsiLbsView &lv = e->lv;
    const float *src = nullptr;
    long cap = 0;
    for (const FitBuf &b : e->table.bufs)
        if (b.name && !strcmp(name, b.name)) { src = (const float *)(e->blob + b.off); cap = (long)(b.bytes / 4); }
    const struct { const char *name; const float *src; long cap; } more[] = {
        {"stats", e->stats_local, 8},
        {"gA", lv.gA, (long)f.B * PSI_JP * 16},
        {"gfeat", lv.gfeat, (long)f.B * lv.m.Kpad},
        {"gl", lv.gl, (long)f.B * lv.m.Npad},
        {"g_vp", lv.g_vp, (long)f.B * lv.m.Npad},
        {"v_posed", lv.v_posed, (long)f.B * lv.m.Npad},
    };
    for (const auto &b : more)
        if (!strcmp(name, b.name)) { src = b.src; cap = b.cap; }
    if (!strcmp(name, "verts") && e->nn_index) {
        hipLaunchKernelGGL(psi_skin_fwd_kernel<PsiSkinNoEpilogue>, dim3(f.nsdfblk, f.B), dim3(PSI_SKIN_BLK), 0, (hipStream_t)stream, lv.m, lv.A,
                           lv.v_posed, f.transl, f.cam, f.B, f.verts, PsiSkinNoEpilogue());
        PSI_CHECK_LAUNCH("skin_fwd_kernel");
    }
    PSI_REQUIRE(src != nullptr, "unknown buffer name");
    PSI_REQUIRE(n_floats <= cap, "buffer is smaller than requested");
    PSI_CHECK_HIP(hipMemcpyAsync(d_out, src, (size_t)n_floats * 4, hipMemcpyDeviceToDevice, (hipStream_t)stream));
    return 0;
}
```

### psi-release_amd/csrc/lbs.hip

```cpp
#include "psi_internal.h"
#include "lbs_device.h"
#include <algorithm>
#include <math.h>
#include <stdlib.h>
#include <vector>
#include <string.h>

typedef float f4 __attribute__((ext_vector_type(4)));
typedef float f2 __attribute__((ext_vector_type(2)));

namespace {

constexpr int JP = PSI_JP;
constexpr int SKIN_BLK = PSI_SKIN_BLK;

}

struct psi_lbs_model {
    LbsDev d;
    void *blob;
};

namespace {

static inline int gv_parts(int B)
{
    int p = 16;
    while (p > 1 && (long)p * B > 1024) p >>= 1;
    return p;
}
struct WsLayout {
    size_t feat, R, Jl, G, A, v_posed, gl, g_vp, gA_part, gfeat_part, gt_part, gA, gfeat, gvbits, total;
    int nsv, nsn, nvb;
};

WsLayout ws_layout(const LbsDev &m, int B)
{
    WsLayout w;
    size_t o = 0;
    auto take = [&](size_t n) { size_t r = o; o += (n + 63) & ~(size_t)63; return r; };
    w.nsv = m.Vpad / 256;
    w.nsn = 256 / (m.Kpad / 64) > 0 ? 256 / (m.Kpad / 64) : 1;
    if (w.nsn > m.Npad / 16) w.nsn = m.Npad / 16;
    w.nvb = m.Vpad / SKIN_BLK;
    w.feat = take((size_t)((B + 31) & ~31) * m.Kpad);
    w.R = take((size_t)B * m.J * 12);
    w.Jl = take((size_t)B * m.J * 3);
    w.G = take((size_t)B * m.J * 12);
    w.A = take((size_t)B * m.J * 12 + PSI_A_TAIL * 12);
    w.v_posed = take((size_t)B * m.Npad);
    w.gl = take((size_t)B * m.Npad);
    w.g_vp = take((size_t)B * m.Npad);
    w.gA_part = take((size_t)w.nsv * B * JP * 16);
    w.gfeat_part = take((size_t)w.nsn * B * m.Kpad);
    w.gt_part = take((size_t)w.nvb * B * 4);
    w.gA = take((size_t)B * JP * 16);
    w.gfeat = take((size_t)B * m.Kpad);
    w.gvbits = take((size_t)B * gv_parts(B));
    w.total = o;
    return w;
}

__global__ __launch_bounds__(64) void pose_fwd_kernel(LbsDev m, const float *__restrict__ betas, const float *__restrict__ pose,
                                                      const float *__restrict__ transl, int B, float *__restrict__ feat,
                                                      float *__restrict__ Rs, float *__restrict__ Jls, float *__restrict__ Gs,
                                                      float *__restrict__ As, float *__restrict__ joints)
{
    const int b = blockIdx.x;
    psi_pose_fwd_body(m, betas + (size_t)b * m.NB, pose + (size_t)b * m.J * 3, transl, B, b, feat, Rs, Jls, Gs, As, joints);
}

typedef _Float16 psi_h8 __attribute__((ext_vector_type(8)));
typedef float psi_f16v __attribute__((ext_vector_type(16)));
typedef unsigned int psi_u4 __attribute__((ext_vector_type(4)));
template <int MTB, int NCH>
__global__ __launch_bounds__(256) __attribute__((amdgpu_waves_per_eu(1, 1))) void blend_fwd_h_kernel(LbsDev m, const float *__restrict__ feat, int B,
                                                                                             float *__restrict__ v_posed)
{
    const int lane = threadIdx.x & 63, w = threadIdx.x >> 6;
    const int tq = blockIdx.x, y = blockIdx.y;
    const int gw = tq * 4 + w;
    if (gw >= m.Npad / 32) return;
    const int bt0 = y * MTB;
    const int li = lane & 31, kh = lane >> 5;
    const int KS = m.Kpad / 16;
    const int nch = NCH ? NCH : m.Kpad / 64;
    const char *dbase = (const char *)m.dirs + (size_t)gw * m.dirs_tile * 4 + (size_t)(kh * 32 + li) * 16;
    const char *fbase = (const char *)feat + (size_t)bt0 * KS * 2048 + (size_t)(kh * 32 + li) * 16;
    auto load_chunk = [&](int ch, psi_u4 (&d)[4][2], psi_u4 (&f)[MTB][4][2]) {
#pragma unroll
        for (int s4 = 0; s4 < 4; s4++)
#pragma unroll
            for (int p = 0; p < 2; p++) {
                d[s4][p] = *(const psi_u4 *)(dbase + (size_t)(ch * 4 + s4) * 2048 + p * 1024);
#pragma unroll
                for (int t = 0; t < MTB; t++) f[t][s4][p] = *(const psi_u4 *)(fbase + ((size_t)t * KS + ch * 4 + s4) * 2048 + p * 1024);
            }
    };
    psi_f16v acc[MTB][2];
#pragma unroll
    for (int t = 0; t < MTB; t++)
#pragma unroll
        for (int c = 0; c < 2; c++)
#pragma unroll
            for (int i = 0; i < 16; i++) acc[t][c][i] = 0.0f;
    auto mfma_chunk = [&](const psi_u4 (&d)[4][2], const psi_u4 (&f)[MTB][4][2]) {
#pragma unroll
        for (int s4 = 0; s4 < 4; s4++)
#pragma unroll
            for (int t = 0; t < MTB; t++) {
                const psi_h8 dh = __builtin_bit_cast(psi_h8, d[s4][0]), dl = __builtin_bit_cast(psi_h8, d[s4][1]);
                const psi_h8 fh = __builtin_bit_cast(psi_h8, f[t][s4][0]), fl = __builtin_bit_cast(psi_h8, f[t][s4][1]);
                acc[t][0] = __builtin_amdgcn_mfma_f32_32x32x16_f16(dh, fh, acc[t][0], 0, 0, 0);
                acc[t][1] = __builtin_amdgcn_mfma_f32_32x32x16_f16(dh, fl, acc[t][1], 0, 0, 0);
                acc[t][1] = __builtin_amdgcn_mfma_f32_32x32x16_f16(dl, fh, acc[t][1], 0, 0, 0);
            }
    };
    if (NCH) {
        psi_u4 d[4][4][2], f[4][MTB][4][2];
#pragma unroll
        for (int ch = 0; ch < 3 && ch < NCH; ch++) {
            load_chunk(ch, d[ch], f[ch]);
            __builtin_amdgcn_sched_barrier(0);
        }
#pragma unroll
        for (int ch = 0; ch < NCH; ch++) {
            if (ch + 3 < NCH) load_chunk(ch + 3, d[(ch + 3) & 3], f[(ch + 3) & 3]);
            __builtin_amdgcn_sched_barrier(0);
            mfma_chunk(d[ch & 3], f[ch & 3]);
            __builtin_amdgcn_sched_barrier(0);
        }
    } else {
        psi_u4 d0[4][2], d1[4][2], f0[MTB][4][2], f1[MTB][4][2];
        load_chunk(0, d0, f0);
        for (int ch = 0; ch < nch; ch += 2) {
            if (ch + 1 < nch) load_chunk(ch + 1, d1, f1);
            __builtin_amdgcn_sched_barrier(0);
            mfma_chunk(d0, f0);
            if (ch + 1 < nch) {
                if (ch + 2 < nch) load_chunk(ch + 2, d0, f0);
                __builtin_amdgcn_sched_barrier(0);
                mfma_chunk(d1, f1);
            }
        }
    }
    const float us = m.dirs_unscale, us2 = m.dirs_unscale * (1.0f / 2048.0f);
#pragma unroll
    for (int g = 0; g < 4; g++) {
        const int n = gw * 32 + 8 * g + 4 * kh;
        const f4 vt = *(const f4 *)(m.v_template + n);
#pragma unroll
        for (int t = 0; t < MTB; t++) {
            const int b = (bt0 + t) * 32 + li;
            f4 o;
#pragma unroll
            for (int e = 0; e < 4; e++) o[e] = vt[e] + __builtin_fmaf(acc[t][1][4 * g + e], us2, acc[t][0][4 * g + e] * us);
            if (b < B) *(f4 *)(v_posed + (size_t)b * m.Npad + n) = o;
        }
    }
}

#ifdef PSI_HEAD_STOPS
// ... 242 lines not shown
    std::vector<float> Wc;
    std::vector<unsigned> Wj;
    {
        int nnz_max = 0;
        for (int v = 0; v < V; v++) {
            int c = 0;
            for (int j = 0; j < J; j++) c += h_weights[(size_t)v * J + j] != 0.0f;
            nnz_max = std::max(nnz_max, c);
        }
        const char *dense = getenv("PSI_LBS_DENSE");
        if (nnz_max <= PSI_WNZ && !(dense && dense[0] == '1')) {
            Wc.assign((size_t)PSI_WNZ * d.Vpad, 0.0f);
            Wj.assign((size_t)(PSI_WNZ / 4) * d.Vpad, 0u);
            for (int v = 0; v < V; v++) {
                int k = 0;
                for (int j = 0; j < J; j++) {
                    float w = h_weights[(size_t)v * J + j];
                    if (w != 0.0f) { Wc[(size_t)k * d.Vpad + v] = w; Wj[(size_t)(k >> 2) * d.Vpad + v] |= (unsigned)j << (8 * (k & 3)); k++; }
                }
            }
        }
    }
    size_t o = 0;
    auto take = [&](size_t bytes) { size_t r = o; o += (bytes + 255) & ~(size_t)255; return r; };
    size_t o_dirs = take(dirs.size() * 4), o_dirs_bh = take(dirs_bh.size() * 4), o_vt = take(vt.size() * 4), o_wt = take(WT.size() * 4), o_wtt = take(WTt.size() * 4), o_jt = take(Jt.size() * 4),
           o_js = take(Js.size() * 4), o_wc = take(Wc.size() * 4 + 4), o_wj = take(Wj.size() * 4 + 4), o_par = take(J * 4), o_lvl = take(J * 4), o_cp = take((J + 1) * 4), o_ci = take(cidx.size() * 4),
           o_jump = take(jump.size() * 4), o_sl = take(sub_list.size()), o_si = take(sub_item.size() * 4), o_sf = take(sub_first.size());
    char *blob = nullptr;
    PSI_CHECK_HIP(hipMalloc((void **)&blob, o));
    std::vector<int> par(h_parents, h_parents + J);
    struct { size_t off; const void *src; size_t bytes; } cp[] = {
        {o_dirs, dirs.data(), dirs.size() * 4}, {o_dirs_bh, dirs_bh.data(), dirs_bh.size() * 4}, {o_vt, vt.data(), vt.size() * 4}, {o_wt, WT.data(), WT.size() * 4}, {o_wtt, WTt.data(), WTt.size() * 4},
        {o_jt, Jt.data(), Jt.size() * 4}, {o_js, Js.data(), Js.size() * 4}, {o_wc, Wc.data(), Wc.size() * 4}, {o_wj, Wj.data(), Wj.size() * 4},
        {o_par, par.data(), (size_t)J * 4},
        {o_lvl, level.data(), (size_t)J * 4}, {o_cp, cptr.data(), (size_t)(J + 1) * 4}, {o_ci, cidx.data(), cidx.size() * 4},
        {o_jump, jump.data(), jump.size() * 4}, {o_sl, sub_list.data(), sub_list.size()}, {o_si, sub_item.data(), sub_item.size() * 4},
        {o_sf, sub_first.data(), sub_first.size()}};
    for (auto &c : cp) {
        if (!c.bytes) continue;
        hipError_t e = hipMemcpy(blob + c.off, c.src, c.bytes, hipMemcpyHostToDevice);
        if (e != hipSuccess) {
            (void)hipFree(blob);
            psi_set_error("hipMemcpy failed: %s", hipGetErrorString(e));
            return (int)e;
        }
    }
    d.dirs = (const float *)(blob + o_dirs);
    d.dirs_bh = (const float *)(blob + o_dirs_bh);
    d.v_template = (const float *)(blob + o_vt);
    d.WT = (const float *)(blob + o_wt);
    d.WTt = (const float *)(blob + o_wtt);
    d.Wc = Wc.empty() ? nullptr : (const float *)(blob + o_wc);
    d.Wj = Wj.empty() ? nullptr : (const unsigned *)(blob + o_wj);
    d.J_t = (const float *)(blob + o_jt);
    d.J_s = (const float *)(blob + o_js);
    d.parents = (const int *)(blob + o_par);
    d.level = (const int *)(blob + o_lvl);
    d.child_ptr = (const int *)(blob + o_cp);
    d.child_idx = (const int *)(blob + o_ci);
    d.jump = (const int *)(blob + o_jump);
    d.sub_list = (const unsigned char *)(blob + o_sl);
    d.sub_item = (const unsigned int *)(blob + o_si);
    d.sub_first = (const unsigned char *)(blob + o_sf);
    psi_lbs_model *mdl = new psi_lbs_model;
    mdl->d = d;
    mdl->blob = blob;
    *out = mdl;
    return 0;
}

extern "C" void psi_lbs_destroy(psi_lbs_model *m)
{
    if (!m) return;
    (void)hipFree(m->blob);
    delete m;
}

extern "C" size_t psi_lbs_workspace_floats(const psi_lbs_model *m, int B)
{
    if (!m || B <= 0) return 0;
    return ws_layout(m->d, B).total;
}

static int lbs_launch_blend(const LbsDev &m, const WsLayout &L, int B, float *ws, hipStream_t st)
{
    const int bgroups = B > 32 ? psi_cdiv(B, 64) : 1;
    const dim3 grid(psi_cdiv(m.Npad / 32, 4), bgroups);
    static const bool loop_form = getenv("PSI_BLEND_FWD_LOOP") && getenv("PSI_BLEND_FWD_LOOP")[0] == '1';
#define PSI_LAUNCH_BLEND(MT_, NCH_) hipLaunchKernelGGL((blend_fwd_h_kernel<MT_, NCH_>), grid, dim3(256), 0, st, m, ws + L.feat, B, ws + L.v_posed)
    const bool k8 = m.Kpad == 512 && !loop_form;
    if (B > 32) { if (k8) PSI_LAUNCH_BLEND(2, 8); else PSI_LAUNCH_BLEND(2, 0); }
    else { if (k8) PSI_LAUNCH_BLEND(1, 8); else PSI_LAUNCH_BLEND(1, 0); }
#undef PSI_LAUNCH_BLEND
    PSI_CHECK_LAUNCH("blend_fwd_kernel");
    psi_mark("blend_fwd_kernel", st);
    return 0;
}

static int lbs_launch_blend_skin(const LbsDev &m, const WsLayout &L, const float *transl, const float *cam_ext, int B, float *verts,
                                 float *ws, hipStream_t st)
{
    int rc = lbs_launch_blend(m, L, B, ws, st);
    if (rc) return rc;
    hipLaunchKernelGGL(psi_skin_fwd_kernel<PsiSkinNoEpilogue>, dim3(m.Vpad / SKIN_BLK, B), dim3(SKIN_BLK), 0, st, m, ws + L.A,
                       ws + L.v_posed, transl, cam_ext, B, verts, PsiSkinNoEpilogue());
    PSI_CHECK_LAUNCH("skin_fwd_kernel");
    psi_mark("skin_fwd_kernel", st);
    return 0;
}

extern "C" int psi_lbs_forward(const psi_lbs_model *mdl, const float *betas, const float *pose, const float *transl,
                               const float *cam_ext, int B, float *verts, float *joints, float *ws, void *stream)
{
    PSI_REQUIRE(mdl && betas && pose && verts && ws, "null pointer");
    PSI_REQUIRE(B > 0 && B <= 16384, "batch size out of range");
    const LbsDev &m = mdl->d;
    WsLayout L = ws_layout(m, B);
    hipStream_t st = (hipStream_t)stream;
    hipLaunchKernelGGL(pose_fwd_kernel, dim3(B), dim3(64), 0, st, m, betas, pose, transl, B, ws + L.feat, ws + L.R, ws + L.Jl,
                       ws + L.G, ws + L.A, joints);
    PSI_CHECK_LAUNCH("pose_fwd_kernel");
    psi_mark("pose_fwd_kernel", st);
    return lbs_launch_blend_skin(m, L, transl, cam_ext, B, verts, ws, st);
}

int psi_lbs_view(const psi_lbs_model *mdl, int B, float *ws, PsiLbsView *out)
{
    PSI_REQUIRE(mdl && ws && out && B > 0, "bad arguments");
    const LbsDev &m = mdl->d;
    WsLayout L = ws_layout(m, B);
    out->m = m;
    out->feat = ws + L.feat; out->R = ws + L.R; out->Jl = ws + L.Jl; out->G = ws + L.G; out->A = ws + L.A;
    out->v_posed = ws + L.v_posed; out->gl = ws + L.gl; out->g_vp = ws + L.g_vp; out->gt_part_w = ws + L.gt_part;
    out->gA_part = ws + L.gA_part; out->gfeat_part = ws + L.gfeat_part; out->gt_part = ws + L.gt_part;
    out->gA = ws + L.gA; out->gfeat = ws + L.gfeat;
    out->nsv = L.nsv; out->nsn = L.nsn; out->nvb = L.nvb;
    return 0;
}

int psi_lbs_counts(const psi_lbs_model *mdl, int B, PsiLbsCounts *out)
{
    PSI_REQUIRE(mdl && out && B > 0, "bad arguments");
    const LbsDev &m = mdl->d;
    const WsLayout L = ws_layout(m, B);
    *out = PsiLbsCounts{L.nsv, L.nsn, m.Kpad, m.Npad, m.Wc != nullptr};
    return 0;
}

int psi_lbs_blend_forward(const psi_lbs_model *mdl, int B, float *ws, hipStream_t st)
{
    const LbsDev &m = mdl->d;
    return lbs_launch_blend(m, ws_layout(m, B), B, ws, st);
}

int psi_lbs_pose_blend_forward(const psi_lbs_model *mdl, const float *betas, const float *pose, const float *transl, int B, float *ws,
                               hipStream_t st)
{
    PSI_REQUIRE(mdl && betas && pose && ws && B > 0, "bad arguments");
    const LbsDev &m = mdl->d;
    WsLayout L = ws_layout(m, B);
    hipLaunchKernelGGL(pose_fwd_kernel, dim3(B), dim3(64), 0, st, m, betas, pose, transl, B, ws + L.feat, ws + L.R, ws + L.Jl,
                       ws + L.G, ws + L.A, (float *)nullptr);
    PSI_CHECK_LAUNCH("pose_fwd_kernel");
    psi_mark("pose_fwd_kernel", st);
    return lbs_launch_blend(m, L, B, ws, st);
}

static int lbs_launch_bwd_joint_parts(const LbsDev &m, const WsLayout &L, int B, float *ws, hipStream_t st);

static int lbs_launch_bwd_partials(const LbsDev &m, const WsLayout &L, const float *grad_verts, const float *cam_ext, int B, float *ws,
                                   hipStream_t st)
{
    if (B >= PSI_SKIN_MB_MIN_B)
        psi_launch_skin_bwd_v_mb(m, ws + L.A, PsiGradFromMemory{grad_verts, m.V}, cam_ext, B, ws + L.gl, ws + L.g_vp, ws + L.gt_part, st);
    else
        hipLaunchKernelGGL(psi_skin_bwd_v_kernel<PsiGradFromMemory>, dim3(m.Vpad / SKIN_BLK, B), dim3(SKIN_BLK), 0, st, m, ws + L.A,
                           PsiGradFromMemory{grad_verts, m.V}, cam_ext, B, ws + L.gl, ws + L.g_vp, ws + L.gt_part);
    PSI_CHECK_LAUNCH("skin_bwd_v_kernel");
    psi_mark("skin_bwd_v_kernel", st);
    return lbs_launch_bwd_joint_parts(m, L, B, ws, st);
}

static int lbs_launch_bwd_joint_parts(const LbsDev &m, const WsLayout &L, int B, float *ws, hipStream_t st)
{
    const int steps = psi_cdiv(m.Npad / 16, L.nsn);
    const int kgroups = m.Kpad / 64;
    const int mt = B > 32 ? 4 : (B > 16 ? 2 : 1);
    const int bgroups = psi_cdiv(B, 16 * mt);
    const int n_blend = kgroups * L.nsn * bgroups;
    static const int nbody_override = psi_ska_nbody_override(SKA_NBODY);
    const int nbody = psi_ska_nbody(psi_cdiv(B, 256 / L.nsv > 0 ? 256 / L.nsv : 1), SKA_NBODY, nbody_override);
    const int grid = n_blend + L.nsv * psi_cdiv(B, nbody);
    const int gvp = gv_parts(B);
    hipLaunchKernelGGL(gv_rowmax_kernel, dim3(gvp, B), dim3(256), 0, st, ws + L.g_vp, m.Npad / 4, (unsigned *)(ws + L.gvbits));
    PSI_CHECK_LAUNCH("gv_rowmax_kernel");
#define PSI_LAUNCH_JOINT(MT_)                                                                                                      \
    hipLaunchKernelGGL(bwd_joint_kernel<MT_>, dim3(grid), dim3(256), 0, st, m, ws + L.g_vp, ws + L.gl, ws + L.v_posed, B, steps,     \
                       ws + L.gfeat_part, ws + L.gA_part, n_blend, kgroups, L.nsn, L.nsv, nbody, (const unsigned *)(ws + L.gvbits), gvp)
    if (mt == 4) PSI_LAUNCH_JOINT(4);
    else if (mt == 2) PSI_LAUNCH_JOINT(2);
    else PSI_LAUNCH_JOINT(1);
#undef PSI_LAUNCH_JOINT
    PSI_CHECK_LAUNCH("bwd_joint_kernel");
    psi_mark("bwd_joint_kernel", st);
    return 0;
}

static int lbs_launch_reduce(const LbsDev &m, const WsLayout &L, int B, float *ws, float *g_transl, hipStream_t st)
{
    long nred = (long)B * JP * 16 + (long)B * m.Kpad + (long)B * 4;
    hipLaunchKernelGGL(reduce_partials_kernel, dim3(psi_cdiv(nred * RSPL, 256)), dim3(256), 0, st, B, m.Kpad, ws + L.gA_part, L.nsv,
                       ws + L.gfeat_part, L.nsn, ws + L.gt_part, L.nvb, ws + L.gA, ws + L.gfeat, g_transl);
    PSI_CHECK_LAUNCH("reduce_partials_kernel");
    psi_mark("reduce_partials_kernel", st);
    return 0;
}

int psi_lbs_backward_joint_parts(const psi_lbs_model *mdl, int B, float *ws, float *g_transl, hipStream_t st, bool reduce)
{
    const LbsDev &m = mdl->d;
    WsLayout L = ws_layout(m, B);
    int rc = lbs_launch_bwd_joint_parts(m, L, B, ws, st);
    if (rc || !reduce) return rc;
    return lbs_launch_reduce(m, L, B, ws, g_transl, st);
}

int psi_lbs_backward_ex(const psi_lbs_model *mdl, const float *grad_verts, const float *betas, const float *pose,
                        const float *cam_ext, int B, float *ws, PsiLbsGradOut out, hipStream_t st)
{
    PSI_REQUIRE(mdl && grad_verts && betas && pose && ws, "null pointer");
    PSI_REQUIRE(B > 0 && B <= 16384, "batch size out of range");
    const LbsDev &m = mdl->d;
    WsLayout L = ws_layout(m, B);
    int rc = lbs_launch_bwd_partials(m, L, grad_verts, cam_ext, B, ws, st);
    if (rc) return rc;
// ... 24 lines not shown
```

### psi-release_amd/csrc/lbs_device.h

```cpp
#pragma once
#ifndef PSI_TRACE
#define PSI_TRACE(lo, hi)
#endif
#ifndef PSI_SSTOP
#define PSI_SSTOP(k)
#endif
#ifndef PSI_PSTOP
#define PSI_PSTOP(k)
#endif
#include <hip/hip_runtime.h>

typedef float psi_f4 __attribute__((ext_vector_type(4)));

constexpr int PSI_JP = 64;
constexpr int PSI_SUB_MAX = PSI_JP * (PSI_JP + 1) / 2;
constexpr int PSI_ITEM_MAX = 2 * PSI_JP;
constexpr int PSI_NJUMP = 6;
constexpr int PSI_WNZ = 8;
constexpr int PSI_A_TAIL = 16;

struct LbsDev {
    int V, J, NB, P, K, Kpad, N, Npad, Vpad, maxlevel, njump;
    int dirs_tile;
    float dirs_unscale;
    const float *dirs, *v_template, *WT, *J_t, *J_s;
    const float *dirs_bh;
    const float *WTt;
    const float *Wc;
    const unsigned *Wj;
    const int *parents, *level, *child_ptr, *child_idx;
    const int *jump;
    const unsigned char *sub_list;
    const unsigned int *sub_item;
    const unsigned char *sub_first;
    int n_sub, n_items;
};

struct PsiLbsView {
    LbsDev m;
    float *feat, *R, *Jl, *G, *A, *v_posed, *gl, *g_vp, *gt_part_w;
    const float *gA_part, *gfeat_part, *gt_part;
    const float *gA, *gfeat;
    int nsv, nsn, nvb;
};

__device__ __forceinline__ void psi_rodrigues(const float *aa, float *R)
{
    float x = aa[0] + 1e-8f, y = aa[1] + 1e-8f, z = aa[2] + 1e-8f;
    float angle = sqrtf(x * x + y * y + z * z);
    float rx = aa[0] / angle, ry = aa[1] / angle, rz = aa[2] / angle;
    float s = sinf(angle), c1 = 1.0f - cosf(angle);
    R[0] = 1.0f + c1 * (-(ry * ry + rz * rz));
    R[1] = s * (-rz) + c1 * (rx * ry);
    R[2] = s * ry + c1 * (rx * rz);
    R[3] = s * rz + c1 * (rx * ry);
    R[4] = 1.0f + c1 * (-(rx * rx + rz * rz));
    R[5] = s * (-rx) + c1 * (ry * rz);
    R[6] = s * (-ry) + c1 * (rx * rz);
    R[7] = s * rx + c1 * (ry * rz);
    R[8] = 1.0f + c1 * (-(rx * rx + ry * ry));
}

__device__ __forceinline__ void psi_pose_fwd_rest(const LbsDev &m, const float *betas_b, float (*sJ)[3])
{
    for (int q = threadIdx.x; q < m.J * 3; q += blockDim.x) {
        float a = m.J_t[q];
        const float *js = m.J_s + (size_t)q * m.NB;
        for (int l = 0; l < m.NB; l++) a += js[l] * betas_b[l];
        (&sJ[0][0])[q] = a;
    }
}

constexpr float PSI_FEAT_SCALE = 16.0f;
__device__ __forceinline__ void psi_feat_store(const LbsDev &m, float *__restrict__ feat, int b, int k, float v)
{
    float x = v * PSI_FEAT_SCALE;
    x = x > 65504.0f ? 65504.0f : (x < -65504.0f ? -65504.0f : x);
    const _Float16 hi = (_Float16)x;
    const _Float16 lo = (_Float16)((x - (float)hi) * 2048.0f);
    _Float16 *o = (_Float16 *)feat + (((size_t)(b >> 5) * (m.Kpad >> 4) + (k >> 4)) * 4 + ((k >> 3) & 1)) * 256 + (size_t)(b & 31) * 8 + (k & 7);
    o[0] = hi;
    o[512] = lo;
}

__device__ __forceinline__ void psi_pose_fwd_rest_store(const LbsDev &m, const float *betas_b, int B, int b, const float (*sJ)[3],
                                                        float *__restrict__ feat, float *__restrict__ Jls)
{
    const int j = threadIdx.x, nthr = blockDim.x;
    for (int q = j; q < m.J * 3; q += nthr) Jls[(size_t)b * m.J * 3 + q] = (&sJ[0][0])[q];
    for (int l = j; l < m.NB; l += nthr) psi_feat_store(m, feat, b, l, betas_b[l]);
    for (int l = m.K + j; l < m.Kpad; l += nthr) psi_feat_store(m, feat, b, l, 0.0f);
}

struct PsiJump { int a[PSI_NJUMP]; };

__device__ __forceinline__ PsiJump psi_load_jump(const LbsDev &m)
{
    PsiJump jp;
#pragma unroll
    for (int r = 0; r < PSI_NJUMP; r++) jp.a[r] = (threadIdx.x < m.J && r < m.njump) ? m.jump[r * PSI_JP + threadIdx.x] : -1;
    return jp;
}

__device__ __forceinline__ void psi_pose_fwd_chain(const LbsDev &m, const float *pose_b, const float *__restrict__ transl, int B, int b,
                                                   const float (*sJ)[3], const PsiJump &jp, float *__restrict__ feat,
                                                   float *__restrict__ Rs, float *__restrict__ Gs, float *__restrict__ As,
                                                   float *__restrict__ joints)
{
    const int j = threadIdx.x;
    __shared__ float sG[PSI_JP][12];
    __shared__ int sJmp[PSI_NJUMP][PSI_JP];
    const bool act = j < m.J;
    float R[9], Jl[3] = {0, 0, 0};
    if (j < PSI_JP)
#pragma unroll
        for (int r = 0; r < PSI_NJUMP; r++) sJmp[r][j] = jp.a[r];
    if (act) {
        psi_rodrigues(pose_b + j * 3, R);
        psi_f4 *Ro = (psi_f4 *)(Rs + ((size_t)b * m.J + j) * 12);
        Ro[0] = psi_f4{R[0], R[1], R[2], 0.0f};
        Ro[1] = psi_f4{R[3], R[4], R[5], 0.0f};
        Ro[2] = psi_f4{R[6], R[7], R[8], 0.0f};
        if (j >= 1)
            for (int e = 0; e < 9; e++) {
                int k = m.NB + (j - 1) * 9 + e;
                psi_feat_store(m, feat, b, k, R[e] - ((e == 0 || e == 4 || e == 8) ? 1.0f : 0.0f));
            }
    }
    __syncthreads();
    float G[12];
    if (act) {
        const int par = jp.a[0];
        for (int c = 0; c < 3; c++) Jl[c] = sJ[j][c];
        for (int r = 0; r < 3; r++) {
            for (int c = 0; c < 3; c++) G[r * 4 + c] = R[r * 3 + c];
            G[r * 4 + 3] = par >= 0 ? Jl[r] - sJ[par][r] : Jl[r];
        }
        for (int e = 0; e < 12; e++) sG[j][e] = G[e];
    }
#pragma nounroll
    for (int r = 0; r < m.njump && j < 64; r++) {
        __builtin_amdgcn_wave_barrier();
        const int a = sJmp[r][j];
        float P[12];
        if (act && a >= 0)
            for (int e = 0; e < 12; e++) P[e] = sG[a][e];
        __builtin_amdgcn_wave_barrier();
        if (act && a >= 0) {
            float N[12];
            for (int q = 0; q < 3; q++) {
                for (int c = 0; c < 3; c++) N[q * 4 + c] = P[q * 4 + 0] * G[0 * 4 + c] + P[q * 4 + 1] * G[1 * 4 + c] + P[q * 4 + 2] * G[2 * 4 + c];
                N[q * 4 + 3] = P[q * 4 + 0] * G[3] + P[q * 4 + 1] * G[7] + P[q * 4 + 2] * G[11] + P[q * 4 + 3];
            }
            for (int e = 0; e < 12; e++) { G[e] = N[e]; sG[j][e] = N[e]; }
        }
    }
    if (act) {
        psi_f4 *Go = (psi_f4 *)(Gs + ((size_t)b * m.J + j) * 12), *Ao = (psi_f4 *)(As + ((size_t)b * m.J + j) * 12);
        for (int r = 0; r < 3; r++) {
            Go[r] = psi_f4{G[r * 4 + 0], G[r * 4 + 1], G[r * 4 + 2], G[r * 4 + 3]};
            Ao[r] = psi_f4{G[r * 4 + 0], G[r * 4 + 1], G[r * 4 + 2],
                           G[r * 4 + 3] - (G[r * 4 + 0] * Jl[0] + G[r * 4 + 1] * Jl[1] + G[r * 4 + 2] * Jl[2])};
        }
        if (joints)
            for (int r = 0; r < 3; r++) joints[((size_t)b * m.J + j) * 3 + r] = G[r * 4 + 3] + (transl ? transl[(size_t)b * 3 + r] : 0.0f);
    }
    if (b == B - 1)
        for (int q = j; q < PSI_A_TAIL * 3; q += blockDim.x) ((psi_f4 *)(As + (size_t)B * m.J * 12))[q] = psi_f4{0.0f, 0.0f, 0.0f, 0.0f};
}


__device__ __forceinline__ void psi_pose_fwd_body(const LbsDev &m, const float *betas_b, const float *pose_b,
                                                  const float *__restrict__ transl, int B, int b, float *__restrict__ feat,
                                                  float *__restrict__ Rs, float *__restrict__ Jls, float *__restrict__ Gs,
                                                  float *__restrict__ As, float *__restrict__ joints)
{
    __shared__ float sJ[PSI_JP][3];
    const PsiJump jp = psi_load_jump(m);
    psi_pose_fwd_rest(m, betas_b, sJ);
    __syncthreads();
    psi_pose_fwd_rest_store(m, betas_b, B, b, sJ, feat, Jls);
    psi_pose_fwd_chain(m, pose_b, transl, B, b, sJ, jp, feat, Rs, Gs, As, joints);
}


constexpr int PSI_POSE_JSP = 8;
struct PsiPoseBwdPre {
    float aa[3], js[PSI_POSE_JSP], G[12], Jl[3], P[12];
    int cp0, cp1, par;
};
struct PsiPoseBwdShared {
    float sX[PSI_JP][12];
    float sS[PSI_JP][12];
    float sP[PSI_ITEM_MAX][12];
    unsigned int sItem[PSI_ITEM_MAX];
    unsigned char sList[PSI_SUB_MAX], sFirst[PSI_JP + 1];
    float sgJ[PSI_JP][3];
    float sgrel[PSI_JP][3];
    int sChild[PSI_JP];
    float sgb[32][32];
};

__device__ __forceinline__ PsiPoseBwdPre psi_pose_bwd_issue(const LbsDev &m, const float *pose_b, const float *__restrict__ Jls,
                                                            const float *__restrict__ Gs, int b, bool want_betas, bool want_pose,
                                                            PsiPoseBwdShared &sh)
{
    const int j = threadIdx.x, nthr = blockDim.x;
    const bool act = j < m.J;
    PsiPoseBwdPre p;
    for (int e = 0; e < 3; e++) p.aa[e] = 0.0f;
    if (act && want_pose)
        for (int e = 0; e < 3; e++) p.aa[e] = pose_b[j * 3 + e];
    constexpr int JSP = PSI_POSE_JSP;
    const int nq = m.J * 3;
    const int npart = m.NB > 0 ? min(32, max(1, nthr / m.NB)) : 1;
    const int per = (nq + npart - 1) / npart;
    const bool par_ok = m.NB <= 32, js_pre = want_betas && par_ok && per <= JSP && j < npart * m.NB;
    const int bpart = m.NB > 0 ? j / m.NB : 0, bl = j - bpart * m.NB;
    for (int i = 0; i < JSP; i++) p.js[i] = 0.0f;
    if (js_pre)
        for (int i = 0; i < JSP; i++) {
            const int q = bpart * per + i;
            if (i < per && q < nq) p.js[i] = m.J_s[(size_t)q * m.NB + bl];
        }
    p.cp0 = act ? m.child_ptr[j] : 0;
    p.cp1 = act ? m.child_ptr[j + 1] : 0;
    p.par = act ? m.parents[j] : -1;
    if (j < m.J - 1) sh.sChild[j] = m.child_idx[j];
    for (int i = j; i < m.n_sub; i += nthr) sh.sList[i] = m.sub_list[i];
    for (int i = j; i < m.n_items; i += nthr) sh.sItem[i] = m.sub_item[i];
    for (int i = j; i <= m.J; i += nthr) sh.sFirst[i] = m.sub_first[i];
    for (int e = 0; e < 12; e++) { p.G[e] = 0.0f; p.P[e] = 0.0f; }
    for (int c = 0; c < 3; c++) p.Jl[c] = 0.0f;
    if (act) {
        const psi_f4 *Gp = (const psi_f4 *)(Gs + ((size_t)b * m.J + j) * 12);
        for (int r = 0; r < 3; r++) {
            const psi_f4 gg = Gp[r];
            for (int c = 0; c < 4; c++) p.G[r * 4 + c] = gg[c];
        }
        for (int c = 0; c < 3; c++) p.Jl[c] = Jls[((size_t)b * m.J + j) * 3 + c];
    }
    if (act && p.par >= 0) {
        const psi_f4 *Pp = (const psi_f4 *)(Gs + ((size_t)b * m.J + p.par) * 12);
        for (int r = 0; r < 3; r++) {
            const psi_f4 pr = Pp[r];
            for (int c = 0; c < 4; c++) p.P[r * 4 + c] = pr[c];
        }
    }
    return p;
}

// ... 703 lines not shown
```

### psi-release_amd/csrc/psi_internal.h

```cpp
#pragma once
#include "psi_common.h"
#include <stdlib.h>

struct psi_lbs_model;

struct PsiStageTimer {
    hipEvent_t ev[48];
    const char *name[48];
    int n;
};
extern thread_local PsiStageTimer *g_psi_timer;
static inline void psi_mark(const char *nm, hipStream_t st)
{
    PsiStageTimer *t = g_psi_timer;
    if (t && t->n < 48) {
        (void)hipEventRecord(t->ev[t->n], st);
        t->name[t->n] = nm;
        t->n++;
    }
}

int psi_nn_contact(const float *verts, long vstride, const int *vid, const float *scene, int B, int n, int m, void *ws,
                   float cconst, float gscale, float *gq, float *fpart, int *idx_out, hipStream_t st);
int psi_nn_contact_fparts(int n);
size_t psi_nn_ws_bytes(int B, int n, int m);

struct psi_nn_index;
int psi_nn_index_contact(const psi_nn_index *ix, const float *verts, long vstride, const int *vid, int B, int n, float cconst,
                         float gscale, float *gq, float *fpart, int *hint, hipStream_t st);
int psi_nn_index_fparts(int n);

struct PsiLbsGradOut {
    float *g_betas;
    float *g_pose;
    float *g_transl;
    float *g_rot;
};
int psi_lbs_backward_ex(const psi_lbs_model *mdl, const float *grad_verts, const float *betas, const float *pose,
                        const float *cam_ext, int B, float *ws, PsiLbsGradOut out, hipStream_t st);
void psi_lbs_dims(const psi_lbs_model *mdl, int *V, int *J, int *NB);
static inline int psi_ska_nbody_override(int limit)
{
    const char *v = getenv("PSI_SKA_NBODY");
    const int n = v ? atoi(v) : 0;
    return n >= 1 && n <= limit ? n : 0;
}
static inline int psi_ska_nbody(int rule, int limit, int override_) { return override_ ? override_ : (rule < limit ? rule : limit); }
struct PsiLbsView;
int psi_lbs_view(const psi_lbs_model *mdl, int B, float *ws, PsiLbsView *out);
struct PsiLbsCounts { int nsv, nsn, Kpad, Npad; bool compressed_weights; };
int psi_lbs_counts(const psi_lbs_model *mdl, int B, PsiLbsCounts *out);
int psi_lbs_blend_forward(const psi_lbs_model *mdl, int B, float *ws, hipStream_t st);
int psi_lbs_pose_blend_forward(const psi_lbs_model *mdl, const float *betas, const float *pose, const float *transl, int B, float *ws,
                               hipStream_t st);
int psi_lbs_backward_joint_parts(const psi_lbs_model *mdl, int B, float *ws, float *g_transl, hipStream_t st,
                                 bool reduce = true);

struct psi_dp_comm;
int psi_dp_world(const psi_dp_comm *c);

bool psi_conv_stem_shape(int Cin, int Cout, int kh, int kw, int stride, int pad);
int psi_conv_stem_forward(const void *x, int x_bf16, const float *w, const float *bias, int N, int H, int W, void *y, int y_bf16, int nterm,
                          hipStream_t st);
size_t psi_conv_stem_wgrad_floats(int N, int H, int W);
int psi_conv_stem_weight_grad(const void *x, int x_bf16, const void *dy, int dy_bf16, int N, int H, int W, float *gw, float *ws, int nterm,
                              hipStream_t st);

int psi_conv3x3_wrw3_ok(int N, int H, int W, int Cin, int Cout);
size_t psi_conv3x3_wrw3_workspace_floats(int N, int H, int W, int Cin, int Cout);
int psi_conv3x3_weight_grad3(const float *x, const float *dy, int N, int H, int W, int Cin, int Cout, float *gw, float *ws, hipStream_t st);
int psi_conv3x3s_ok(int N, int H, int W, int Cin, int Cout);
int psi_conv3x3s_forward(const float *x, const void *wp, const float *bias, int N, int H, int W, int Cin, int Cout, float *y, int reversed_taps, hipStream_t st);
```

### psi-release_amd/fitting.py

```python
from __future__ import annotations

import ctypes
import os
import pickle

import numpy as np
import torch
import torch.nn.functional as F
import torch.optim as optim

from . import body_model, dist as psi_dist, hip, ops, scene_io
from .geometry import BodyParamParser, GeometryTransformer
from .vposer import load_vposer


HAS_FUSED_ENGINE = True


def expand_cam_ext(cam_ext, B):
    if cam_ext.dim() != 3 or tuple(cam_ext.shape[1:]) != (4, 4) or cam_ext.shape[0] not in (1, B):
        raise ValueError('cam_ext must be [%d,4,4] or [1,4,4], got %s' % (B, tuple(cam_ext.shape)))
    return cam_ext.expand(B, 4, 4).contiguous() if cam_ext.shape[0] != B else cam_ext


# ... 358 lines not shown
        w3, b3 = f32(sd['bodyprior_dec_out.weight']), f32(sd['bodyprior_dec_out.bias'])
        if w1.shape != (512, 32) or w2.shape != (512, 512) or w3.shape != (126, 512):
            raise hip.PsiHipError('the fused engine expects VPoser(512, 32, [1,21,3])')
        lhc, rhc = f32(bm.left_hand_components.cpu().numpy()), f32(bm.right_hand_components.cpu().numpy())
        pm = f32(bm.pose_mean.cpu().numpy())
        vid = np.ascontiguousarray(op.contact_vertex_ids().cpu().numpy(), dtype=np.int32)
        gmin, gmax = f32(op.s_grid_min_batch.cpu().numpy().reshape(3)), f32(op.s_grid_max_batch.cpu().numpy().reshape(3))
        world = op.dp_world() if hasattr(op, 'dp_world') else 1
        self.world = world
        if world > 1:
            psi_dist.assert_equal_across_ranks(op.batch_size, 'per-rank batch size')
        cfg = hip.FitConfig(B=op.batch_size, n_contact=len(vid), m_scene=op.s_verts.shape[1], D=op.s_sdf.shape[1],
                            align_corners=int(bool(op.align_corners)), world_size=world, num_pca_comps=lhc.shape[0],
                            max_history=4096, nn_mode=1 if op.nn_mode == 'kdtree' else 0, w_rec=op.weight_loss_rec, w_vposer=op.weight_loss_vposer,
                            w_contact=op.weight_contact, w_collision=op.weight_collision, contact_const=op.contact_const,
                            lr=op.init_lr_h, beta1=0.9, beta2=0.999, eps=1e-8, lr_d=float(op.init_lr_h), beta1_d=0.9, beta2_d=0.999,
                            independent_bodies=int(bool(getattr(op, 'independent_bodies', False))),
                            concurrent_engines=int(getattr(op, 'concurrent_engines', 1)))
        self.concurrent_engines = int(getattr(op, 'concurrent_engines', 1))
        self._keep = (op.s_verts, op.s_sdf)
        h = ctypes.c_void_p()
        p = lambda a: a.ctypes.data_as(ctypes.c_void_p)
        tab = getattr(op, '_scene_tab', None)
        self.n_scenes = len(tab) if tab and (len(tab) > 1 or getattr(op, 'scene_table_engine', False)) else 0
        with torch.cuda.device(dev):
            if self.n_scenes:
                arr = (hip.FitScene * self.n_scenes)()
                for s_, sc in zip(arr, tab):
                    s_.d_verts, s_.d_sdf, s_.m, s_.D = hip.ptr(sc['verts']), hip.ptr(sc['sdf']), sc['verts'].shape[0], sc['sdf'].shape[0]
                    s_.gmin[:], s_.gmax[:] = [float(v) for v in sc['gmin']], [float(v) for v in sc['gmax']]
                self._keep = tuple(tab)
                hip.check(hip.lib().psi_fit_create_scenes(ctypes.byref(h), bm.lbs_model.handle, ctypes.byref(cfg), p(w1), p(b1), p(w2), p(b2),
                                                          p(w3), p(b3), p(lhc), p(rhc), p(pm), p(vid), arr, self.n_scenes), 'psi_fit_create_scenes')
            else:
                hip.check(hip.lib().psi_fit_create(ctypes.byref(h), bm.lbs_model.handle, ctypes.byref(cfg), p(w1), p(b1), p(w2), p(b2),
                                                   p(w3), p(b3), p(lhc), p(rhc), p(pm), p(vid), hip.ptr(op.s_verts), hip.ptr(op.s_sdf),
                                                   p(gmin), p(gmax)), 'psi_fit_create')
        self.handle = h
        self.stream = torch.cuda.Stream(device=dev)
        self.stats = torch.zeros(8, device=dev)
        self.max_history = 4096

    def set_scene_slots(self, slot):
        if not self.n_scenes:
            return
        self._slots = slot.contiguous()
        self.stream.wait_stream(torch.cuda.current_stream())
        hip.check(hip.lib().psi_fit_set_scene_slots(self.handle, hip.ptr(self._slots), self.stream.cuda_stream), 'psi_fit_set_scene_slots')

    def set_problem(self, xhr, x_init, cam, reset):
        B = self.op.batch_size
        if tuple(xhr.shape) != (B, 75) or tuple(x_init.shape) != (B, 75):
            raise ValueError('FusedEngine was built for batch_size=%d: expected body vectors of shape (%d, 75), got %s / %s (a generated-body '
                             'pkl must hold batch_size rows)' % (B, B, tuple(xhr.shape), tuple(x_init.shape)))
        cam = expand_cam_ext(cam, B)
        if self.n_scenes:
            self.set_scene_slots(self.op._slot_dev)
        cur = torch.cuda.current_stream()
        self.stream.wait_stream(cur)
        self._args = (xhr.contiguous(), x_init.contiguous(), cam.contiguous())
        hip.check(hip.lib().psi_fit_set_problem(self.handle, hip.ptr(self._args[0]), hip.ptr(self._args[1]), hip.ptr(self._args[2]),
                                                int(bool(reset)), self.stream.cuda_stream), 'psi_fit_set_problem')

    def iterate(self, n, use_graph=True):
        L = hip.lib()
        if self.world == 1 and not (os.environ.get('PSI_FORCE_DP_PATH') == '1' and torch.distributed.is_initialized()):
            hip.check(L.psi_fit_iterate(self.handle, n, int(bool(use_graph)), self.stream.cuda_stream), 'psi_fit_iterate')
            return
        import torch.distributed as tdist
        if tdist.get_backend() == 'nccl' and os.environ.get('PSI_DP_PYTHON_LOOP') != '1':
            hip.check(L.psi_fit_iterate_dp(self.handle, psi_dist.rccl_comm(), n, int(bool(use_graph)), hip.ptr(self.stats), self.stream.cuda_stream),
                      'psi_fit_iterate_dp')
            return
        use_graph = bool(use_graph) and (getattr(self.op, 'dp_use_graph', False) or os.environ.get('PSI_DP_GRAPH') == '1')
        with torch.cuda.stream(self.stream):
            for _ in range(n):
                hip.check(L.psi_fit_forward(self.handle, hip.ptr(self.stats), int(bool(use_graph)), self.stream.cuda_stream), 'psi_fit_forward')
                tdist.all_reduce(self.stats, op=tdist.ReduceOp.SUM)
                hip.check(L.psi_fit_backward_step(self.handle, hip.ptr(self.stats), int(bool(use_graph)), self.stream.cuda_stream), 'psi_fit_backward_step')

    def dp_mode(self):
        return int(hip.lib().psi_fit_dp_mode(self.handle))

    def watchdog(self):
        if self.world > 1 or os.environ.get('PSI_FORCE_DP_PATH') == '1':
            limit = float(os.environ.get('PSI_DP_WATCHDOG_S', '60'))
            hip.check(hip.lib().psi_stream_wait(self.stream.cuda_stream, int(limit * 1000)), 'psi_stream_wait (data-parallel watchdog)')

    def read(self, n_hist=0):
        op = self.op
        self.watchdog()
        x = torch.empty(op.batch_size, 75, device=op.device)
        hist = torch.empty(max(n_hist, 1), 4, device=op.device)
        step = ctypes.c_int(0)
        hip.check(hip.lib().psi_fit_read(self.handle, hip.ptr(x), hip.ptr(hist), n_hist, ctypes.byref(step), self.stream.cuda_stream),
                  'psi_fit_read')
        torch.cuda.current_stream().wait_stream(self.stream)
        return x, hist[:n_hist], step.value

    def read_losses(self, adam_step):
        out = torch.empty(4, device=self.op.device)
        self.watchdog()
        hip.check(hip.lib().psi_fit_read_losses(self.handle, int(adam_step), hip.ptr(out), self.stream.cuda_stream), 'psi_fit_read_losses')
        self.stream.synchronize()
        return out

    def profile(self, n_rep=20):
        names = ctypes.create_string_buffer(48 * 48)
        ms = (ctypes.c_float * 48)()
        n = ctypes.c_int(0)
        hip.check(hip.lib().psi_fit_profile(self.handle, n_rep, names, 48, ms, 48, ctypes.byref(n), self.stream.cuda_stream),
                  'psi_fit_profile')
        out = []
        for i in range(n.value):
            out.append((names.raw[i * 48:(i + 1) * 48].split(b'\0')[0].decode(), float(ms[i])))
        return out

    def buffer(self, name, shape):
        out = torch.empty(*shape, device=self.op.device)
        hip.check(hip.lib().psi_fit_copy_buffer(self.handle, name.encode(), hip.ptr(out), out.numel(), self.stream.cuda_stream),
                  'psi_fit_copy_buffer')
        self.stream.synchronize()
        return out

    def __del__(self):
        try:
            if getattr(self, 'handle', None):
                torch.cuda.synchronize()
                hip.lib().psi_fit_destroy(self.handle)
                self.handle = None
        except Exception:
            pass


class _FusedRunner:

    def __init__(self, op, xhr, cam):
        self.op = op
        if getattr(op, '_fused', None) is None:
            op._fused = FusedEngine(op)
            first = True
        else:
            first = False
        self.eng = op._fused
        self.eng.set_problem(xhr, op.xhr_rec.data, cam, reset=op.reset_optimizer and not first)
        _, _, self.step0 = self.eng.read(0)
        self.n = 0

    def step(self):
        self.eng.iterate(1, self.op.use_graph)
        self.n += 1

    def steps(self, n):
        self.eng.iterate(n, self.op.use_graph)
        self.n += n

    def restart(self):
        xhr, _, cam = self.eng._args
        self.eng.set_problem(xhr, xhr, cam, reset=True)
        self.step0, self.n = 0, 0

    def last_losses(self):
        idx = self.step0 + self.n
        if idx < 1:
            return [float('nan')] * 4
        return [float(v) for v in self.eng.read_losses(idx).cpu()]
# ... 55 lines not shown
```

### psi-release_amd/hip.py

```python
from __future__ import annotations

import ctypes
import os

import torch

_PKG = os.path.dirname(os.path.abspath(__file__))
LIB_PATH = os.environ.get('PSI_HIP_LIB') or os.path.join(
    _PKG, 'lib', 'libpsi_hip_fma.so' if os.environ.get('PSI_CHAMFER_FMA') == '1' else 'libpsi_hip.so')
_lib = None

c_void_p, c_int, c_long, c_size_t, c_float, c_double = ctypes.c_void_p, ctypes.c_int, ctypes.c_long, ctypes.c_size_t, ctypes.c_float, ctypes.c_double

SIGNATURES = {
    'psi_last_error': (ctypes.c_char_p, []),
    'psi_version': (c_int, []),
    'psi_device_info': (c_int, [c_void_p] * 4),
    'psi_chamfer_arith_mode': (c_int, []),
    'psi_chamfer_workspace_bytes': (c_size_t, [c_int] * 3),
    'psi_chamfer_forward': (c_int, [c_void_p, c_void_p, c_int, c_int, c_int, c_void_p, c_void_p, c_void_p, c_void_p,
                                    c_void_p, c_void_p]),
    'psi_chamfer_backward': (c_int, [c_void_p] * 8 + [c_int] * 3 + [c_void_p]),
    'psi_scratch_release': (c_int, [c_void_p, c_int]),
    'psi_nn_index_create': (c_int, [c_void_p, c_void_p, c_int]),
    'psi_nn_index_destroy': (None, [c_void_p]),
    'psi_nn_index_query': (c_int, [c_void_p, c_void_p, c_int, c_int, c_void_p, c_void_p, c_void_p, c_void_p]),
    'psi_nn_index_set_create': (c_int, [c_void_p, c_void_p, c_int]),
    'psi_nn_index_set_destroy': (None, [c_void_p]),
    'psi_nn_index_set_query': (c_int, [c_void_p, c_void_p, c_void_p, c_int, c_int, c_void_p, c_void_p, c_void_p]),
    'psi_sdf_sample_forward': (c_int, [c_void_p] * 5 + [c_int] * 5 + [c_void_p] * 3),
    'psi_sdf_sample_backward': (c_int, [c_void_p, c_void_p, c_int, c_int, c_void_p, c_void_p]),
    'psi_sdf_penetration_stats': (c_int, [c_void_p, c_long, c_void_p, c_void_p]),
    'psi_lbs_create': (c_int, [c_void_p] * 7 + [c_int] * 3),
    'psi_lbs_destroy': (None, [c_void_p]),
    'psi_lbs_workspace_floats': (c_size_t, [c_void_p, c_int]),
    'psi_lbs_forward': (c_int, [c_void_p] * 5 + [c_int] + [c_void_p] * 4),
    'psi_lbs_backward': (c_int, [c_void_p] * 5 + [c_int] + [c_void_p] * 5),
    'psi_linear_workspace_floats': (c_size_t, [c_int] * 3),
    'psi_linear_forward': (c_int, [c_void_p, c_int, c_void_p, c_void_p, c_void_p, c_int, c_int, c_int, c_int, c_float, c_void_p, c_void_p, c_void_p,
                                   c_void_p]),
    'psi_linear_forward3': (c_int, [c_void_p, c_int, c_void_p, c_void_p, c_void_p, c_int, c_int, c_int, c_int, c_float, c_void_p, c_void_p, c_void_p,
                                    c_void_p]),
    'psi_linear_backward_workspace_floats': (c_size_t, [c_int, c_int, c_int]),
    'psi_linear_backward': (c_int, [c_void_p, c_void_p, c_void_p, c_int, c_void_p, c_int, c_int, c_int, c_float, c_void_p, c_void_p, c_void_p,
                                    c_void_p, c_void_p]),
    'psi_linear_backward3': (c_int, [c_void_p, c_void_p, c_void_p, c_void_p, c_int, c_int, c_int, c_float, c_void_p, c_void_p, c_void_p, c_void_p, c_void_p]),
    'psi_adam_step': (c_int, [c_void_p] * 5 + [c_int, c_void_p, c_void_p] + [c_double] * 5 + [c_void_p]),
    'psi_fit_create': (c_int, [c_void_p] * 17),
    'psi_fit_destroy': (None, [c_void_p]),
    'psi_fit_create_scenes': (c_int, [c_void_p] * 14 + [c_int]),
    'psi_fit_set_scene_slots': (c_int, [c_void_p, c_void_p, c_void_p]),
    'psi_fit_scene_count': (c_int, [c_void_p]),
    'psi_fit_set_problem': (c_int, [c_void_p] * 4 + [c_int, c_void_p]),
    'psi_fit_forward': (c_int, [c_void_p, c_void_p, c_int, c_void_p]),
    'psi_fit_backward_step': (c_int, [c_void_p, c_void_p, c_int, c_void_p]),
    'psi_fit_iterate': (c_int, [c_void_p, c_int, c_int, c_void_p]),
    'psi_bn_workspace_floats': (c_size_t, [c_long, c_int]),
    'psi_bn_forward': (c_int, [c_void_p] * 7 + [c_long, c_int, c_int, c_float, c_float] + [c_void_p] * 5),
    'psi_bn_backward': (c_int, [c_void_p] * 6 + [c_long, c_int, c_int] + [c_void_p] * 6),
    'psi_bn_forward_t': (c_int, [c_void_p, c_int] + [c_void_p] * 6 + [c_long, c_int, c_int, c_float, c_float] + [c_void_p] * 4 + [c_int, c_void_p]),
    'psi_bn_backward_t': (c_int, [c_void_p, c_int] + [c_void_p] * 6 + [c_long, c_int, c_int] + [c_void_p] * 6),
    'psi_maxpool3x3s2_forward_t': (c_int, [c_void_p, c_int, c_int, c_int, c_int, c_int, c_void_p, c_void_p, c_void_p]),
    'psi_maxpool3x3s2_backward_t': (c_int, [c_void_p, c_int, c_void_p, c_int, c_int, c_int, c_int, c_void_p, c_void_p]),
    'psi_conv2d_supported': (c_int, [c_int] * 6),
    'psi_conv2d_forward': (c_int, [c_void_p, c_int, c_void_p, c_void_p] + [c_int] * 9 + [c_void_p, c_int, c_int, c_void_p]),
    'psi_conv2d_input_grad': (c_int, [c_void_p, c_int, c_void_p] + [c_int] * 9 + [c_void_p, c_int, c_int, c_void_p]),
    'psi_conv2d_prepared_ok': (c_int, [c_int] * 6),
    'psi_conv2d_prepare_weight': (c_int, [c_void_p] + [c_int] * 5 + [c_void_p, c_void_p, c_void_p]),
    'psi_conv2d_forward_p': (c_int, [c_void_p, c_int, c_void_p, c_void_p] + [c_int] * 9 + [c_void_p, c_int, c_int, c_void_p]),
    'psi_conv2d_input_grad_p': (c_int, [c_void_p, c_int, c_void_p] + [c_int] * 9 + [c_void_p, c_int, c_int, c_void_p]),
    'psi_conv2d_wgrad_workspace_floats': (c_size_t, [c_int] * 9),
    'psi_conv2d_weight_grad': (c_int, [c_void_p, c_int, c_void_p, c_int] + [c_int] * 9 + [c_void_p, c_void_p, c_int, c_void_p]),
    'psi_conv3x3_supported': (c_int, [c_int] * 4),
    'psi_conv3x3_forward': (c_int, [c_void_p, c_void_p, c_void_p, c_int, c_int, c_int, c_int, c_int, c_void_p, c_void_p]),
    'psi_conv3x3_wrw_workspace_floats': (c_size_t, [c_int] * 5),
    'psi_conv3x3_weight_grad': (c_int, [c_void_p, c_void_p, c_int, c_int, c_int, c_int, c_int, c_void_p, c_void_p, c_void_p]),
    'psi_conv3x3_rotate_weight': (c_int, [c_void_p, c_int, c_int, c_void_p, c_void_p]),
    'psi_conv3x3_prepare_weight': (c_int, [c_void_p, c_int, c_int, c_void_p, c_void_p, c_void_p]),
    'psi_maxpool3x3s2_forward': (c_int, [c_void_p, c_int, c_int, c_int, c_int, c_void_p, c_void_p, c_void_p]),
    'psi_maxpool3x3s2_backward': (c_int, [c_void_p, c_void_p, c_int, c_int, c_int, c_int, c_void_p, c_void_p]),
    'psi_cvae_target': (c_int, [c_void_p, c_void_p, c_void_p, c_int, c_void_p, c_void_p]),
    'psi_cvae_losses_workspace_floats': (c_size_t, []),
    'psi_cvae_losses_forward': (c_int, [c_void_p] * 7 + [c_int, c_void_p, c_void_p, c_int, c_int, c_float, c_float, c_float, c_float,
                                        c_void_p, c_void_p, c_void_p, c_void_p, c_void_p]),
    'psi_cvae_losses_backward': (c_int, [c_void_p] * 7 + [c_int, c_void_p, c_void_p, c_int, c_int, c_float, c_float, c_float, c_float,
                                         c_void_p, c_void_p, c_void_p, c_void_p, c_void_p, c_void_p, c_void_p, c_void_p, c_void_p, c_void_p]),
    'psi_scene_losses_workspace_floats': (c_size_t, []),
    'psi_scene_losses_forward': (c_int, [c_void_p, c_long, c_void_p, c_long, c_float, c_float, c_float, c_void_p, c_void_p, c_void_p, c_void_p]),
    'psi_scene_losses_backward': (c_int, [c_void_p] * 7 + [c_long, c_void_p, c_void_p, c_void_p, c_int, c_int, c_int, c_float, c_float, c_float,
                                          c_void_p, c_void_p, c_void_p]),
    'psi_contact_slot_chain': (c_int, [c_void_p, c_int, c_void_p, c_void_p]),
    'psi_fit_dp_mode': (c_int, [c_void_p]),
    'psi_stream_wait': (c_int, [c_void_p, c_int]),
    'psi_dp_unique_id': (c_int, [c_void_p]),
    'psi_dp_comm_create': (c_int, [c_void_p, c_void_p, c_int, c_int]),
    'psi_dp_comm_destroy': (None, [c_void_p]),
    'psi_dp_comm_info': (c_int, [c_void_p, c_void_p, c_void_p, c_void_p]),
    'psi_dp_allreduce_sum': (c_int, [c_void_p, c_void_p, c_int, c_void_p]),
    'psi_fit_iterate_dp': (c_int, [c_void_p, c_void_p, c_int, c_int, c_void_p, c_void_p]),
    'psi_fit_read': (c_int, [c_void_p, c_void_p, c_void_p, c_int, c_void_p, c_void_p]),
    'psi_fit_read_losses': (c_int, [c_void_p, c_int, c_void_p, c_void_p]),
    'psi_fit_decode_forward': (c_int, [c_void_p, c_void_p, c_void_p, c_void_p, c_void_p]),
    'psi_fit_decode_backward': (c_int, [c_void_p, c_void_p, c_void_p, c_void_p]),
    'psi_fit_profile': (c_int, [c_void_p, c_int, c_void_p, c_int, c_void_p, c_int, c_void_p, c_void_p]),
    'psi_fit_copy_buffer': (c_int, [c_void_p, ctypes.c_char_p, c_void_p, c_long, c_void_p]),
    'psi_lbs_sdf_counts': (c_int, [c_void_p] * 5 + [c_int] + [c_void_p] * 4 + [c_int] * 3 + [c_void_p] * 3),
    'psi_kmeans_create': (c_int, [c_void_p, c_void_p, c_int, c_int, c_void_p, c_int, c_int, c_float]),
    'psi_kmeans_destroy': (None, [c_void_p]),
    'psi_kmeans_iterate': (c_int, [c_void_p, c_int, c_void_p]),
    'psi_kmeans_read': (c_int, [c_void_p] * 7),
    'psi_vq': (c_int, [c_void_p, c_int, c_int, c_void_p, c_int, c_void_p, c_void_p, c_void_p]),
    'psi_raster_mesh_create': (c_int, [c_void_p] * 4 + [c_int, c_int]),
    'psi_raster_mesh_destroy': (None, [c_void_p]),
    'psi_raster_workspace_bytes': (c_size_t, [c_int] * 4),
    'psi_raster_render': (c_int, [c_void_p] * 3 + [c_int, c_int, c_int, c_float] + [c_void_p] * 6),
    'psi_raster_bodies_create': (c_int, [c_void_p] * 2 + [c_int, c_int]),
    'psi_raster_bodies_destroy': (None, [c_void_p]),
    'psi_raster_bodies_normals': (c_int, [c_void_p] * 2 + [c_int] + [c_void_p] * 2),
    'psi_raster_bodies_workspace_bytes': (c_size_t, [c_int] * 5),
    'psi_raster_bodies_render': (c_int, [c_void_p] * 4 + [c_int] + [c_void_p] * 3 + [c_int] + [c_void_p] * 2 + [c_int] * 3 + [c_float] + [c_void_p] * 2
                                 + [c_float] * 3 + [c_int] + [c_void_p] * 9),
    'psi_mesh_sdf_create': (c_int, [c_void_p] * 3 + [c_int, c_int]),
    'psi_mesh_sdf_destroy': (None, [c_void_p]),
    'psi_mesh_sdf_info': (c_int, [c_void_p, c_void_p]),
    'psi_mesh_sdf_compute': (c_int, [c_void_p] * 3 + [c_int, c_int, c_void_p, c_void_p]),
    'psi_mesh_sdf_count_pairs': (c_int, [c_void_p] * 3 + [c_int, c_int, c_void_p, c_void_p]),
    'psi_mesh_winding_compute': (c_int, [c_void_p] * 3 + [c_int, c_float, c_int, c_void_p, c_void_p]),
    'psi_mesh_winding_count': (c_int, [c_void_p] * 3 + [c_int, c_float, c_int, c_void_p, c_void_p]),
    'psi_mesh_sdf_apply_sign': (c_int, [c_void_p, c_float, c_void_p, ctypes.c_longlong, c_void_p]),
    'psi_snapshot_canvas_workspace_bytes': (c_size_t, [c_int]),
    'psi_snapshot_canvas': (c_int, [c_void_p] * 2 + [c_int] * 5 + [c_float] * 2 + [c_void_p] * 9),
    'psi_mesh_cloud_count': (c_int, [c_void_p] * 2 + [c_int] * 2 + [c_float] + [c_void_p] * 5),
    'psi_mesh_cloud_rows': (c_int, [c_void_p] * 2 + [c_int] * 2 + [c_float, c_void_p, ctypes.c_longlong] + [c_void_p] * 3),
    'psi_mesh_cloud_emit': (c_int, [c_void_p] * 2 + [c_int] * 2 + [c_float] + [c_void_p] * 4 + [ctypes.c_longlong] * 2 + [c_void_p] * 5),
    'psi_mesh_cloud_winners': (c_int, [c_void_p] * 3 + [ctypes.c_longlong] + [c_void_p] * 2),
    'psi_mesh_cloud_compact': (c_int, [c_void_p] * 4 + [ctypes.c_longlong] * 2 + [c_void_p] * 3),
    'psi_flood_fill': (c_int, [c_void_p] + [c_int] * 3 + [c_void_p, c_int] + [c_void_p] * 3),
    'psi_mesh_orient_votes': (c_int, [c_void_p] * 2 + [ctypes.c_longlong, c_void_p, c_int, c_void_p, c_int] + [c_void_p] * 3 + [c_int, c_float]
                              + [c_void_p] * 2),
    'psi_body_overlap_create': (c_int, [c_void_p] * 2 + [c_int] * 2),
    'psi_body_overlap_destroy': (None, [c_void_p]),
    'psi_body_overlap_info': (c_int, [c_void_p] * 2),
    'psi_body_overlap_workspace_bytes': (c_size_t, [ctypes.c_longlong, c_int]),
    'psi_body_overlap_boxes': (c_int, [c_void_p] * 2 + [c_int] + [c_void_p] * 3),
    'psi_body_overlap_count': (c_int, [c_void_p] * 3 + [c_int] + [c_void_p] * 3),
    'psi_body_overlap_emit': (c_int, [c_void_p] * 3 + [c_int] + [c_void_p] * 4 + [ctypes.c_longlong] * 2 + [c_void_p] * 3),
    'psi_body_overlap_wind': (c_int, [c_void_p] * 2 + [c_int, c_void_p, ctypes.c_longlong, c_void_p, ctypes.c_longlong, c_void_p, c_size_t, c_void_p]),
    'psi_body_overlap_decide': (c_int, [c_void_p, c_int, c_void_p, ctypes.c_longlong, c_void_p, c_size_t] + [c_void_p] * 4),
    'psi_body_depth_workspace_bytes': (c_size_t, [ctypes.c_longlong, c_int]),
    'psi_body_depth_nearest': (c_int, [c_void_p] * 2 + [c_int, c_void_p, ctypes.c_longlong, c_void_p, ctypes.c_longlong, c_void_p, c_size_t, c_void_p]),
    'psi_body_depth_finish': (c_int, [c_void_p] * 2 + [c_int, c_void_p, ctypes.c_longlong, c_void_p, c_size_t] + [c_void_p] * 6),
    'psi_body_depth_pairs': (c_int, [c_void_p, c_int, c_void_p, ctypes.c_longlong] + [c_void_p] * 8),
    'psi_body_depth_grad_rows': (c_int, [c_void_p, c_int, c_void_p, ctypes.c_longlong] + [c_void_p] * 5 + [c_int] + [c_void_p] * 3),
    'psi_segment_sum3': (c_int, [c_void_p] * 3 + [ctypes.c_longlong, c_void_p, ctypes.c_longlong, c_void_p]),
    'psi_surface_crossings_face_order': (c_int, [c_void_p, c_int, c_int, c_void_p, c_void_p]),
    'psi_surface_crossings_create': (c_int, [c_void_p] * 2 + [c_int] * 2 + [c_void_p] * 3 + [c_int]),
    'psi_surface_crossings_destroy': (None, [c_void_p]),
    'psi_surface_crossings_info': (c_int, [c_void_p] * 2),
    'psi_surface_crossings_boxes': (c_int, [c_void_p] * 2 + [c_int] + [c_void_p] * 4),
    'psi_surface_crossings_tiles': (c_int, [c_void_p] * 2 + [c_int] * 2 + [c_void_p] * 4 + [ctypes.c_longlong] + [c_void_p] * 2),
    'psi_surface_crossings_test': (c_int, [c_void_p] * 2 + [c_int, c_void_p, ctypes.c_longlong] + [c_void_p] * 2 + [ctypes.c_longlong]
                                   + [c_void_p] * 4),
    'psi_surface_crossings_finish': (c_int, [c_void_p, c_int] + [c_void_p] * 4 + [ctypes.c_longlong] + [c_void_p] * 9),
    'psi_crossing_field_eval': (c_int, [c_void_p] * 2 + [c_int, c_void_p, ctypes.c_longlong, c_float] + [c_void_p] * 3),
    'psi_crossing_field_pairs': (c_int, [c_void_p, c_int, c_void_p, ctypes.c_longlong] + [c_void_p] * 7),
    'psi_crossing_field_grad_rows': (c_int, [c_void_p] * 2 + [c_int, c_void_p, ctypes.c_longlong, c_float] + [c_void_p] * 4),
    'psi_body_separate_pose': (c_int, [c_void_p] * 4 + [c_int] * 2 + [c_void_p] * 2),
    'psi_body_separate_wrench': (c_int, [c_void_p] * 3 + [c_int] * 2 + [c_void_p] * 3),
    'psi_body_separate_step': (c_int, [c_void_p, c_int] + [c_void_p] * 6 + [c_int] + [c_float] * 7 + [c_void_p]),
    'psi_body_separate_scene': (c_int, [c_void_p] * 6 + [c_int] * 4 + [c_float] + [c_void_p] * 6),
}


class FitConfig(ctypes.Structure):
    _fields_ = [('B', c_int), ('n_contact', c_int), ('m_scene', c_int), ('D', c_int), ('align_corners', c_int),
# ... 62 lines not shown
```

Measured before the change: 11800.

## Move kinematic chain from head kernel into extra blend-kernel workgroups

When the head runs as a multi-block cluster, the head kernel now only computes Rodrigues rotations and rest joints. The serial kinematic-chain transform composition moves into extra workgroups appended to the blend kernel, one wave per body. The aim is to take the latency-bound chain off the head's critical path and run it alongside the blend GEMM. Rodrigues and chain arithmetic are rewritten with explicit FMA and contraction disabled, presumably to match the reference rounding. The cost is extra launch configuration and shared memory in the blend kernel, plus more ordering constraints between the kernels.

After: 12030 (median of 6 runs). 1.9% higher.

```diff
diff --git a/include/psi_hip.h b/include/psi_hip.h
--- a/include/psi_hip.h
+++ b/include/psi_hip.h
@@ -104,6 +104,7 @@
 int psi_dp_allreduce_sum(psi_dp_comm *comm, float *d_buf, int n, void *stream);
 int psi_fit_iterate_dp(psi_fit_engine *engine, psi_dp_comm *comm, int n_iter, int use_graph, float *d_stats, void *stream);
 int psi_fit_dp_mode(const psi_fit_engine *engine);
+int psi_fit_chain_mode(const psi_fit_engine *engine);
 int psi_stream_wait(void *stream, int timeout_ms);
 
 int psi_fit_profile(psi_fit_engine *engine, int n_rep, char *h_names, int name_stride, float *h_ms, int max_stages,
diff --git a/psi-release_amd/csrc/chain_plan.h b/psi-release_amd/csrc/chain_plan.h
--- /dev/null
+++ b/psi-release_amd/csrc/chain_plan.h
@@ -0,0 +1,29 @@
+#pragma once
+
+#if defined(__HIPCC__) || defined(__CUDACC__)
+#define PSI_CHAIN_HD __host__ __device__
+#else
+#define PSI_CHAIN_HD
+#endif
+
+constexpr int PSI_CHAIN_WG_MAX = 8;
+constexpr int PSI_CHAIN_WAVES = 4;
+
+struct PsiChainPlan {
+    int n_links_wg;
+    int bodies_per_wave;
+};
+
+PSI_CHAIN_HD inline PsiChainPlan psi_chain_plan(int B, int hc, int n_stream, int grid_y, int cus)
+{
+    const PsiChainPlan off = {0, 0};
+    if (B < 1 || hc <= 1 || grid_y != 1) return off;
+    PsiChainPlan p;
+    p.bodies_per_wave = (B + 31) / 32;
+    const int per_wg = PSI_CHAIN_WAVES * p.bodies_per_wave;
+    p.n_links_wg = (B + per_wg - 1) / per_wg;
+    if (p.n_links_wg > PSI_CHAIN_WG_MAX || p.n_links_wg > cus - n_stream) return off;
+    return p;
+}
+
+PSI_CHAIN_HD inline int psi_chain_first_body(const PsiChainPlan &p, int g, int w) { return (g * PSI_CHAIN_WAVES + w) * p.bodies_per_wave; }
diff --git a/psi-release_amd/csrc/fit.hip b/psi-release_amd/csrc/fit.hip
--- a/psi-release_amd/csrc/fit.hip
+++ b/psi-release_amd/csrc/fit.hip
@@ -4,6 +4,8 @@
 #define PSI_SSTOP(k) do { if (psi_dbg_sstop == (k)) return; } while (0)
 __device__ int psi_dbg_pstop;
 #define PSI_PSTOP(k) do { if (psi_dbg_pstop == (k)) asm volatile("s_endpgm"); } while (0)
+__device__ int psi_dbg_cstop;
+#define PSI_CSTOP() do { if (psi_dbg_cstop) asm volatile("s_endpgm"); } while (0)
 #define PSI_TRACE(lo, hi) PsiBlockTrace trace_((lo), (hi))
 __device__ unsigned long long psi_dbg_tl[4 * 8192];
 struct PsiBlockTrace {
@@ -28,6 +30,7 @@
 }
 #endif
 #include "lbs_device.h"
+#include "chain_plan.h"
 #include "lbs_joint_device.h"
 #include "sdf_device.h"
 #include "nnindex_device.h"
@@ -243,7 +246,7 @@
     return __uint_as_float((unsigned)w);
 }
 
-template <int C>
+template <int C, bool LINKS_IN_HEAD>
 __global__ __launch_bounds__(HB) void head_fwd_kernel(FitDev f, PsiLbsView lv)
 {
     constexpr int NS = NH / C;
@@ -285,7 +288,7 @@
         if (t < 22)
             for (int e = 0; e < 3; e++) pm[e] = f.pose_mean[t * 3 + e];
         if (t < 128) b3v = f.b3[t];
-        jp = psi_load_jump(lv.m);
+        if (LINKS_IN_HEAD) jp = psi_load_jump(lv.m);
     }
     __syncthreads();
     HSTOP(1);
@@ -403,7 +406,12 @@
     }
     __syncthreads();
     HSTOP(7);
-    psi_pose_fwd_chain(lv.m, spose, nullptr, f.B, b, sJ, jp, lv.feat, lv.R, lv.G, lv.A, nullptr);
+    if constexpr (LINKS_IN_HEAD) {
+        psi_pose_fwd_chain(lv.m, spose, nullptr, f.B, b, sJ, jp, lv.feat, lv.R, lv.G, lv.A, nullptr);
+    } else {
+        float R[9];
+        psi_pose_fwd_rot(lv.m, spose, b, t, lv.feat, lv.R, R);
+    }
     HSTOP(8);
     psi_pose_fwd_rest_store(lv.m, sbetas, f.B, b, sJ, lv.feat, lv.Jl);
     for (int i = t; i < f.J * 3; i += HB) f.pose[(size_t)b * f.J * 3 + i] = spose[i];
@@ -1437,7 +1445,7 @@
 constexpr int GRAPH_UNROLL = PSI_GRAPH_UNROLL;
 
 struct FitKnobs {
-    bool split_scene, keep_verts, no_fused_bwd, sdf_linear, scene_skin_first, bwdv_mb, no_pen_skip, bwd_pf1;
+    bool split_scene, keep_verts, no_fused_bwd, sdf_linear, scene_skin_first, bwdv_mb, no_pen_skip, bwd_pf1, chain_in_head;
     int head_cluster, skin_nb, ska_nbody, search_lanes;
 #ifdef PSI_HEAD_STOPS
     int head_stop, tail_stop, skin_stop;
@@ -1454,6 +1462,7 @@
     k.no_fused_bwd = is("PSI_FIT_FUSED_BWD", '0');
     k.no_pen_skip = is("PSI_FIT_PEN_SKIP", '0');
     k.bwd_pf1 = is("PSI_FIT_BWD_PF", '1');
+    k.chain_in_head = is("PSI_FIT_CHAIN_IN_HEAD", '1');
     k.sdf_linear = is("PSI_SDF_LINEAR", '1');
     k.scene_skin_first = is("PSI_SCENE_ORDER", '1');
     k.bwdv_mb = is("PSI_BWDV_MB", '1');
@@ -1481,9 +1490,10 @@
     int hc;
     int gv_sps;
     PsiStreamSplit split;
+    PsiChainPlan chain;
 };
 
-static FitModes fit_decide(const psi_fit_config *cfg, const FitKnobs &knobs, int J, int ncp3, const PsiLbsCounts &mc)
+static FitModes fit_decide(const psi_fit_config *cfg, const FitKnobs &knobs, int J, int ncp3, const PsiLbsCounts &mc, int cus)
 {
     FitModes d = {};
     d.self_skin = cfg->nn_mode == 1 && J <= PSI_JP - 8 && psikd::kd_qpb(psikd::LPQ_OPS) == psikd::kd_qpb(2);
@@ -1499,6 +1509,7 @@
     d.fused_bwd = d.merged_scene && !knobs.no_fused_bwd && d.split.nsn_c > 0;
     d.skin_nb = cfg->B > 128 && !mc.compressed_weights ? 2 : 1;
     if (knobs.skin_nb) d.skin_nb = knobs.skin_nb;
+    d.chain = knobs.chain_in_head ? PsiChainPlan{0, 0} : psi_chain_plan(cfg->B, d.hc, mc.blend_wg, mc.blend_gy, cus);
     return d;
 }
 
@@ -1652,15 +1663,29 @@
     bool dp_no_graph;
 };
 
+template <bool LINKS_IN_HEAD>
 static void launch_head_fwd(const FitDev &f, const PsiLbsView &lv, hipStream_t st)
 {
     const dim3 g(f.B * f.hc), blk(HB);
     switch (f.hc) {
-    case 8: hipLaunchKernelGGL(head_fwd_kernel<8>, g, blk, 0, st, f, lv); break;
-    case 4: hipLaunchKernelGGL(head_fwd_kernel<4>, g, blk, 0, st, f, lv); break;
-    case 2: hipLaunchKernelGGL(head_fwd_kernel<2>, g, blk, 0, st, f, lv); break;
-    default: hipLaunchKernelGGL(head_fwd_kernel<1>, g, blk, 0, st, f, lv); break;
-    }
+    case 8: hipLaunchKernelGGL((head_fwd_kernel<8, LINKS_IN_HEAD>), g, blk, 0, st, f, lv); break;
+    case 4: hipLaunchKernelGGL((head_fwd_kernel<4, LINKS_IN_HEAD>), g, blk, 0, st, f, lv); break;
+    case 2: hipLaunchKernelGGL((head_fwd_kernel<2, LINKS_IN_HEAD>), g, blk, 0, st, f, lv); break;
+    default: hipLaunchKernelGGL((head_fwd_kernel<1, true>), g, blk, 0, st, f, lv); break;
+    }
+}
+
+static int fit_head_blend(psi_fit_engine *e, hipStream_t st)
+{
+    const FitDev &f = e->d;
+    const PsiChainPlan &cp = e->mode.chain;
+    const bool role = cp.n_links_wg > 0 && f.hc > 1;
+    if (role) launch_head_fwd<false>(f, e->lv, st);
+    else launch_head_fwd<true>(f, e->lv, st);
+    PSI_CHECK_LAUNCH("head_fwd_kernel");
+    psi_mark("head_fwd_kernel", st);
+    return role ? psi_lbs_blend_forward_links(e->lbs, f.B, e->lbs_ws, cp.n_links_wg, cp.bodies_per_wave, st)
+                : psi_lbs_blend_forward(e->lbs, f.B, e->lbs_ws, st);
 }
 
 template <bool ADAM>
@@ -1740,10 +1765,7 @@
 static int fit_forward(psi_fit_engine *e, float *stats, hipStream_t st, FitStats who)
 {
     FitDev &f = e->d;
-    launch_head_fwd(f, e->lv, st);
-    PSI_CHECK_LAUNCH("head_fwd_kernel");
-    psi_mark("head_fwd_kernel", st);
-    int rc = psi_lbs_blend_forward(e->lbs, f.B, e->lbs_ws, st);
+    int rc = fit_head_blend(e, st);
     if (rc) return rc;
     float gscale = f.w_contact / ((f.indep ? 1.0f : (float)f.B * (float)f.world) * (float)f.n_c);
     if (e->nn_index && e->mode.merged_scene) {
@@ -1904,7 +1926,10 @@
     f.nsv_c = f.ncp / 256;
     f.scene = d_scene_verts;
     f.sdf = d_sdf;
-    const FitModes &mode = e->mode = fit_decide(cfg, knobs, J, f.ncp3, mc);
+    int dev = 0, cus = 0;
+    PSI_CHECK_HIP(hipGetDevice(&dev));
+    PSI_CHECK_HIP(hipDeviceGetAttribute(&cus, hipDeviceAttributeMultiprocessorCount, dev));
+    const FitModes &mode = e->mode = fit_decide(cfg, knobs, J, f.ncp3, mc, cus);
     f.hc = mode.hc;
     f.gv_sps = mode.gv_sps;
     f.fused_bwd = mode.fused_bwd ? 1 : 0;
@@ -1915,6 +1940,8 @@
     f.stop_t = knobs.tail_stop;
     (void)hipMemcpyToSymbol(HIP_SYMBOL(psi_dbg_sstop), &knobs.skin_stop, sizeof(int));
     (void)hipMemcpyToSymbol(HIP_SYMBOL(psi_dbg_pstop), &f.stop_t, sizeof(int));
+    const int cstop = knobs.head_stop == 9;
+    (void)hipMemcpyToSymbol(HIP_SYMBOL(psi_dbg_cstop), &cstop, sizeof(int));
 #endif
     const size_t B = (size_t)f.B;
     std::vector<float> W1T((size_t)NZ * NH), W2T((size_t)NH * NH), W3T((size_t)NH * 128, 0.0f), b3p(128, 0.0f);
@@ -2284,6 +2311,11 @@
     return eager(n_iter);
 }
 
+extern "C" int psi_fit_chain_mode(const psi_fit_engine *e)
+{
+    return e && e->mode.chain.n_links_wg > 0 && e->d.hc > 1 ? 1 : 0;
+}
+
 extern "C" int psi_fit_dp_mode(const psi_fit_engine *e)
 {
     if (!e || !e->dp_warm) return 0;
@@ -2297,9 +2329,7 @@
     hipStream_t st = (hipStream_t)stream;
     PSI_CHECK_HIP(hipMemcpyAsync(f.x, d_x75, fit_x_bytes(f), hipMemcpyDeviceToDevice, st));
     PSI_CHECK_HIP(hipMemcpyAsync(f.cam, d_cam_ext, fit_cam_bytes(f), hipMemcpyDeviceToDevice, st));
-    launch_head_fwd(f, e->lv, st);
-    PSI_CHECK_LAUNCH("head_fwd_kernel");
-    int rc = psi_lbs_blend_forward(e->lbs, f.B, e->lbs_ws, st);
+    int rc = fit_head_blend(e, st);
     if (rc) return rc;
     hipLaunchKernelGGL(psi_skin_fwd_kernel<PsiSkinNoEpilogue>, dim3(f.nsdfblk, f.B), dim3(PSI_SKIN_BLK), 0, st, e->lv.m, e->lv.A,
                        e->lv.v_posed, f.transl, f.cam, f.B, d_verts, PsiSkinNoEpilogue());
@@ -2414,6 +2444,10 @@
         {"gl", lv.gl, (long)f.B * lv.m.Npad},
         {"g_vp", lv.g_vp, (long)f.B * lv.m.Npad},
         {"v_posed", lv.v_posed, (long)f.B * lv.m.Npad},
+        {"R", lv.R, (long)f.B * lv.m.J * 12},
+        {"G", lv.G, (long)f.B * lv.m.J * 12},
+        {"A", lv.A, (long)f.B * lv.m.J * 12 + PSI_A_TAIL * 12},
+        {"feat", lv.feat, (long)((f.B + 31) & ~31) * lv.m.Kpad},
     };
     for (const auto &b : more)
         if (!strcmp(name, b.name)) { src = b.src; cap = b.cap; }
diff --git a/psi-release_amd/csrc/lbs.hip b/psi-release_amd/csrc/lbs.hip
--- a/psi-release_amd/csrc/lbs.hip
+++ b/psi-release_amd/csrc/lbs.hip
@@ -1,5 +1,6 @@
 #include "psi_internal.h"
 #include "lbs_device.h"
+#include "chain_plan.h"
 #include <algorithm>
 #include <math.h>
 #include <stdlib.h>
@@ -73,11 +74,48 @@
 typedef _Float16 psi_h8 __attribute__((ext_vector_type(8)));
 typedef float psi_f16v __attribute__((ext_vector_type(16)));
 typedef unsigned int psi_u4 __attribute__((ext_vector_type(4)));
-template <int MTB, int NCH>
+template <bool LINKS> struct PsiLinksArgs {};
+template <> struct PsiLinksArgs<true> {
+    const float *Rs, *Jls;
+    float *Gs, *As;
+    int n_stream, bpw;
+};
+template <int MTB, int NCH, bool LINKS = false>
 __global__ __launch_bounds__(256) __attribute__((amdgpu_waves_per_eu(1, 1))) void blend_fwd_h_kernel(LbsDev m, const float *__restrict__ feat, int B,
-                                                                                             float *__restrict__ v_posed)
+                                                                                             float *__restrict__ v_posed, PsiLinksArgs<LINKS> la)
 {
     const int lane = threadIdx.x & 63, w = threadIdx.x >> 6;
+    if constexpr (LINKS) {
+        if ((int)blockIdx.x >= la.n_stream) {
+            __shared__ float sGw[4][PSI_JP][12];
+            __shared__ int sJmpw[4][PSI_NJUMP][PSI_JP];
+            const int b0 = psi_chain_first_body(PsiChainPlan{0, la.bpw}, (int)blockIdx.x - la.n_stream, w);
+            if (b0 >= B) return;
+            PsiJump jp;
+#pragma unroll
+            for (int r = 0; r < PSI_NJUMP; r++) {
+                jp.a[r] = (lane < m.J && r < m.njump) ? m.jump[r * PSI_JP + lane] : -1;
+                sJmpw[w][r][lane] = jp.a[r];
+            }
+            for (int b = b0; b < b0 + la.bpw && b < B; b++) {
+                float R[9];
+#pragma unroll
+                for (int e = 0; e < 9; e++) R[e] = 0.0f;
+                if (lane < m.J) {
+                    const psi_f4 *Rp = (const psi_f4 *)(la.Rs + ((size_t)b * m.J + lane) * 12);
+#pragma unroll
+                    for (int r = 0; r < 3; r++) {
+                        const psi_f4 rr = Rp[r];
+                        R[r * 3 + 0] = rr[0]; R[r * 3 + 1] = rr[1]; R[r * 3 + 2] = rr[2];
+                    }
+                }
+                psi_pose_fwd_links(m, nullptr, B, b, lane, 64, R, (const float (*)[3])(la.Jls + (size_t)b * m.J * 3), jp, sGw[w], sJmpw[w], la.Gs, la.As,
+                                   nullptr);
+                __builtin_amdgcn_wave_barrier();
+            }
+            return;
+        }
+    }
     const int tq = blockIdx.x, y = blockIdx.y;
     const int gw = tq * 4 + w;
     if (gw >= m.Npad / 32) return;
@@ -486,16 +524,31 @@
     return ws_layout(m->d, B).total;
 }
 
-static int lbs_launch_blend(const LbsDev &m, const WsLayout &L, int B, float *ws, hipStream_t st)
+static inline dim3 lbs_blend_grid(const LbsDev &m, int B)
 {
     const int bgroups = B > 32 ? psi_cdiv(B, 64) : 1;
-    const dim3 grid(psi_cdiv(m.Npad / 32, 4), bgroups);
+    return dim3(psi_cdiv(m.Npad / 32, 4), bgroups);
+}
+
+static int lbs_launch_blend(const LbsDev &m, const WsLayout &L, int B, float *ws, hipStream_t st, int n_links_wg = 0, int bpw = 0)
+{
+    dim3 grid = lbs_blend_grid(m, B);
     static const bool loop_form = getenv("PSI_BLEND_FWD_LOOP") && getenv("PSI_BLEND_FWD_LOOP")[0] == '1';
-#define PSI_LAUNCH_BLEND(MT_, NCH_) hipLaunchKernelGGL((blend_fwd_h_kernel<MT_, NCH_>), grid, dim3(256), 0, st, m, ws + L.feat, B, ws + L.v_posed)
     const bool k8 = m.Kpad == 512 && !loop_form;
-    if (B > 32) { if (k8) PSI_LAUNCH_BLEND(2, 8); else PSI_LAUNCH_BLEND(2, 0); }
-    else { if (k8) PSI_LAUNCH_BLEND(1, 8); else PSI_LAUNCH_BLEND(1, 0); }
+    if (n_links_wg > 0) {
+        PSI_REQUIRE(grid.y == 1 && bpw >= 1 && (long)n_links_wg * 4 * bpw >= B, "the links role needs a one-row grid and a wave for every body");
+        const PsiLinksArgs<true> la = {ws + L.R, ws + L.Jl, ws + L.G, ws + L.A, (int)grid.x, bpw};
+        grid.x += n_links_wg;
+#define PSI_LAUNCH_BLEND_LINKS(MT_, NCH_) hipLaunchKernelGGL((blend_fwd_h_kernel<MT_, NCH_, true>), grid, dim3(256), 0, st, m, ws + L.feat, B, ws + L.v_posed, la)
+        if (B > 32) { if (k8) PSI_LAUNCH_BLEND_LINKS(2, 8); else PSI_LAUNCH_BLEND_LINKS(2, 0); }
+        else { if (k8) PSI_LAUNCH_BLEND_LINKS(1, 8); else PSI_LAUNCH_BLEND_LINKS(1, 0); }
+#undef PSI_LAUNCH_BLEND_LINKS
+    } else {
+#define PSI_LAUNCH_BLEND(MT_, NCH_) hipLaunchKernelGGL((blend_fwd_h_kernel<MT_, NCH_>), grid, dim3(256), 0, st, m, ws + L.feat, B, ws + L.v_posed, PsiLinksArgs<false>{})
+        if (B > 32) { if (k8) PSI_LAUNCH_BLEND(2, 8); else PSI_LAUNCH_BLEND(2, 0); }
+        else { if (k8) PSI_LAUNCH_BLEND(1, 8); else PSI_LAUNCH_BLEND(1, 0); }
 #undef PSI_LAUNCH_BLEND
+    }
     PSI_CHECK_LAUNCH("blend_fwd_kernel");
     psi_mark("blend_fwd_kernel", st);
     return 0;
@@ -547,7 +600,8 @@
     PSI_REQUIRE(mdl && out && B > 0, "bad arguments");
     const LbsDev &m = mdl->d;
     const WsLayout L = ws_layout(m, B);
-    *out = PsiLbsCounts{L.nsv, L.nsn, m.Kpad, m.Npad, m.Wc != nullptr};
+    const dim3 bg = lbs_blend_grid(m, B);
+    *out = PsiLbsCounts{L.nsv, L.nsn, m.Kpad, m.Npad, m.Wc != nullptr, (int)bg.x, (int)bg.y};
     return 0;
 }
 
@@ -555,6 +609,13 @@
 {
     const LbsDev &m = mdl->d;
     return lbs_launch_blend(m, ws_layout(m, B), B, ws, st);
+}
+
+int psi_lbs_blend_forward_links(const psi_lbs_model *mdl, int B, float *ws, int n_links_wg, int bodies_per_wave, hipStream_t st)
+{
+    PSI_REQUIRE(mdl && ws && B > 0 && n_links_wg > 0 && bodies_per_wave > 0, "bad arguments");
+    const LbsDev &m = mdl->d;
+    return lbs_launch_blend(m, ws_layout(m, B), B, ws, st, n_links_wg, bodies_per_wave);
 }
 
 int psi_lbs_pose_blend_forward(const psi_lbs_model *mdl, const float *betas, const float *pose, const float *transl, int B, float *ws,
diff --git a/psi-release_amd/csrc/lbs_device.h b/psi-release_amd/csrc/lbs_device.h
--- a/psi-release_amd/csrc/lbs_device.h
+++ b/psi-release_amd/csrc/lbs_device.h
@@ -4,6 +4,9 @@
 #endif
 #ifndef PSI_SSTOP
 #define PSI_SSTOP(k)
+#endif
+#ifndef PSI_CSTOP
+#define PSI_CSTOP()
 #endif
 #ifndef PSI_PSTOP
 #define PSI_PSTOP(k)
@@ -46,19 +49,21 @@
 
 __device__ __forceinline__ void psi_rodrigues(const float *aa, float *R)
 {
+#pragma clang fp contract(off)
     float x = aa[0] + 1e-8f, y = aa[1] + 1e-8f, z = aa[2] + 1e-8f;
-    float angle = sqrtf(x * x + y * y + z * z);
+    float angle = sqrtf(__builtin_fmaf(y, y, x * x) + z * z);
     float rx = aa[0] / angle, ry = aa[1] / angle, rz = aa[2] / angle;
     float s = sinf(angle), c1 = 1.0f - cosf(angle);
-    R[0] = 1.0f + c1 * (-(ry * ry + rz * rz));
-    R[1] = s * (-rz) + c1 * (rx * ry);
-    R[2] = s * ry + c1 * (rx * rz);
-    R[3] = s * rz + c1 * (rx * ry);
-    R[4] = 1.0f + c1 * (-(rx * rx + rz * rz));
-    R[5] = s * (-rx) + c1 * (ry * rz);
-    R[6] = s * (-ry) + c1 * (rx * rz);
-    R[7] = s * rx + c1 * (ry * rz);
-    R[8] = 1.0f + c1 * (-(rx * rx + ry * ry));
+    const float cxy = c1 * (rx * ry), cxz = c1 * (rx * rz), cyz = c1 * (ry * rz);
+    R[0] = 1.0f - c1 * __builtin_fmaf(ry, ry, rz * rz);
+    R[1] = cxy - rz * s;
+    R[2] = __builtin_fmaf(ry, s, cxz);
+    R[3] = __builtin_fmaf(rz, s, cxy);
+    R[4] = __builtin_fmaf(-(rx * rx + rz * rz), c1, 1.0f);
+    R[5] = cyz - rx * s;
+    R[6] = cxz - ry * s;
+    R[7] = __builtin_fmaf(rx, s, cyz);
+    R[8] = __builtin_fmaf(-__builtin_fmaf(ry, ry, rx * rx), c1, 1.0f);
 }
 
 __device__ __forceinline__ void psi_pose_fwd_rest(const LbsDev &m, const float *betas_b, float (*sJ)[3])
@@ -102,20 +107,9 @@
     return jp;
 }
 
-__device__ __forceinline__ void psi_pose_fwd_chain(const LbsDev &m, const float *pose_b, const float *__restrict__ transl, int B, int b,
-                                                   const float (*sJ)[3], const PsiJump &jp, float *__restrict__ feat,
-                                                   float *__restrict__ Rs, float *__restrict__ Gs, float *__restrict__ As,
-                                                   float *__restrict__ joints)
-{
-    const int j = threadIdx.x;
-    __shared__ float sG[PSI_JP][12];
-    __shared__ int sJmp[PSI_NJUMP][PSI_JP];
-    const bool act = j < m.J;
-    float R[9], Jl[3] = {0, 0, 0};
-    if (j < PSI_JP)
-#pragma unroll
-        for (int r = 0; r < PSI_NJUMP; r++) sJmp[r][j] = jp.a[r];
-    if (act) {
+__device__ __forceinline__ void psi_pose_fwd_rot(const LbsDev &m, const float *pose_b, int b, int j, float *feat, float *Rs, float (&R)[9])
+{
+    if (j < m.J) {
         psi_rodrigues(pose_b + j * 3, R);
         psi_f4 *Ro = (psi_f4 *)(Rs + ((size_t)b * m.J + j) * 12);
         Ro[0] = psi_f4{R[0], R[1], R[2], 0.0f};
@@ -127,14 +121,22 @@
                 psi_feat_store(m, feat, b, k, R[e] - ((e == 0 || e == 4 || e == 8) ? 1.0f : 0.0f));
             }
     }
-    __syncthreads();
+}
+
+__device__ __forceinline__ void psi_pose_fwd_links(const LbsDev &m, const float *transl, int B, int b, int j, int nthr, const float (&R)[9],
+                                                   const float (*J3)[3], const PsiJump &jp, float (*sG)[12], int (*sJmp)[PSI_JP], float *Gs,
+                                                   float *As, float *joints)
+{
+#pragma clang fp contract(off)
+    const bool act = j < m.J;
+    float Jl[3] = {0, 0, 0};
     float G[12];
     if (act) {
         const int par = jp.a[0];
-        for (int c = 0; c < 3; c++) Jl[c] = sJ[j][c];
+        for (int c = 0; c < 3; c++) Jl[c] = J3[j][c];
         for (int r = 0; r < 3; r++) {
             for (int c = 0; c < 3; c++) G[r * 4 + c] = R[r * 3 + c];
-            G[r * 4 + 3] = par >= 0 ? Jl[r] - sJ[par][r] : Jl[r];
+            G[r * 4 + 3] = par >= 0 ? Jl[r] - J3[par][r] : Jl[r];
         }
         for (int e = 0; e < 12; e++) sG[j][e] = G[e];
     }
@@ -149,8 +151,11 @@
         if (act && a >= 0) {
             float N[12];
             for (int q = 0; q < 3; q++) {
-                for (int c = 0; c < 3; c++) N[q * 4 + c] = P[q * 4 + 0] * G[0 * 4 + c] + P[q * 4 + 1] * G[1 * 4 + c] + P[q * 4 + 2] * G[2 * 4 + c];
-                N[q * 4 + 3] = P[q * 4 + 0] * G[3] + P[q * 4 + 1] * G[7] + P[q * 4 + 2] * G[11] + P[q * 4 + 3];
+                const float p0 = P[q * 4 + 0], p1 = P[q * 4 + 1], p2 = P[q * 4 + 2];
+                for (int c = 0; c < 2; c++) N[q * 4 + c] = __builtin_fmaf(p2, G[8 + c], __builtin_fmaf(p0, G[c], p1 * G[4 + c]));
+                N[q * 4 + 2] = p2 * G[10] + (q < 2 ? __builtin_fmaf(p0, G[2], p1 * G[6]) : p0 * G[2] + p1 * G[6]);
+                N[q * 4 + 3] = P[q * 4 + 3] + (q < 2 ? __builtin_fmaf(p2, G[11], __builtin_fmaf(p1, G[7], p0 * G[3]))
+                                                    : p2 * G[11] + __builtin_fmaf(p0, G[3], p1 * G[7]));
             }
             for (int e = 0; e < 12; e++) { G[e] = N[e]; sG[j][e] = N[e]; }
         }
@@ -160,13 +165,31 @@
         for (int r = 0; r < 3; r++) {
             Go[r] = psi_f4{G[r * 4 + 0], G[r * 4 + 1], G[r * 4 + 2], G[r * 4 + 3]};
             Ao[r] = psi_f4{G[r * 4 + 0], G[r * 4 + 1], G[r * 4 + 2],
-                           G[r * 4 + 3] - (G[r * 4 + 0] * Jl[0] + G[r * 4 + 1] * Jl[1] + G[r * 4 + 2] * Jl[2])};
+                           G[r * 4 + 3] - (G[r * 4 + 2] * Jl[2] + __builtin_fmaf(G[r * 4 + 0], Jl[0], G[r * 4 + 1] * Jl[1]))};
         }
         if (joints)
             for (int r = 0; r < 3; r++) joints[((size_t)b * m.J + j) * 3 + r] = G[r * 4 + 3] + (transl ? transl[(size_t)b * 3 + r] : 0.0f);
     }
     if (b == B - 1)
-        for (int q = j; q < PSI_A_TAIL * 3; q += blockDim.x) ((psi_f4 *)(As + (size_t)B * m.J * 12))[q] = psi_f4{0.0f, 0.0f, 0.0f, 0.0f};
+        for (int q = j; q < PSI_A_TAIL * 3; q += nthr) ((psi_f4 *)(As + (size_t)B * m.J * 12))[q] = psi_f4{0.0f, 0.0f, 0.0f, 0.0f};
+}
+
+__device__ __forceinline__ void psi_pose_fwd_chain(const LbsDev &m, const float *pose_b, const float *__restrict__ transl, int B, int b,
+                                                   const float (*sJ)[3], const PsiJump &jp, float *__restrict__ feat,
+                                                   float *__restrict__ Rs, float *__restrict__ Gs, float *__restrict__ As,
+                                                   float *__restrict__ joints)
+{
+    const int j = threadIdx.x;
+    __shared__ float sG[PSI_JP][12];
+    __shared__ int sJmp[PSI_NJUMP][PSI_JP];
+    float R[9];
+    if (j < PSI_JP)
+#pragma unroll
+        for (int r = 0; r < PSI_NJUMP; r++) sJmp[r][j] = jp.a[r];
+    psi_pose_fwd_rot(m, pose_b, b, j, feat, Rs, R);
+    PSI_CSTOP();
+    __syncthreads();
+    psi_pose_fwd_links(m, transl, B, b, j, blockDim.x, R, sJ, jp, sG, sJmp, Gs, As, joints);
 }
 
 
diff --git a/psi-release_amd/csrc/psi_internal.h b/psi-release_amd/csrc/psi_internal.h
--- a/psi-release_amd/csrc/psi_internal.h
+++ b/psi-release_amd/csrc/psi_internal.h
@@ -48,9 +48,10 @@
 static inline int psi_ska_nbody(int rule, int limit, int override_) { return override_ ? override_ : (rule < limit ? rule : limit); }
 struct PsiLbsView;
 int psi_lbs_view(const psi_lbs_model *mdl, int B, float *ws, PsiLbsView *out);
-struct PsiLbsCounts { int nsv, nsn, Kpad, Npad; bool compressed_weights; };
+struct PsiLbsCounts { int nsv, nsn, Kpad, Npad; bool compressed_weights; int blend_wg, blend_gy; };
 int psi_lbs_counts(const psi_lbs_model *mdl, int B, PsiLbsCounts *out);
 int psi_lbs_blend_forward(const psi_lbs_model *mdl, int B, float *ws, hipStream_t st);
+int psi_lbs_blend_forward_links(const psi_lbs_model *mdl, int B, float *ws, int n_links_wg, int bodies_per_wave, hipStream_t st);
 int psi_lbs_pose_blend_forward(const psi_lbs_model *mdl, const float *betas, const float *pose, const float *transl, int B, float *ws,
                                hipStream_t st);
 int psi_lbs_backward_joint_parts(const psi_lbs_model *mdl, int B, float *ws, float *g_transl, hipStream_t st,
diff --git a/psi-release_amd/fitting.py b/psi-release_amd/fitting.py
--- a/psi-release_amd/fitting.py
+++ b/psi-release_amd/fitting.py
@@ -464,6 +464,9 @@
     def dp_mode(self):
         return int(hip.lib().psi_fit_dp_mode(self.handle))
 
+    def chain_mode(self):
+        return int(hip.lib().psi_fit_chain_mode(self.handle))
+
     def watchdog(self):
         if self.world > 1 or os.environ.get('PSI_FORCE_DP_PATH') == '1':
             limit = float(os.environ.get('PSI_DP_WATCHDOG_S', '60'))
diff --git a/psi-release_amd/hip.py b/psi-release_amd/hip.py
--- a/psi-release_amd/hip.py
+++ b/psi-release_amd/hip.py
@@ -91,6 +91,7 @@
                                           c_void_p, c_void_p, c_void_p]),
     'psi_contact_slot_chain': (c_int, [c_void_p, c_int, c_void_p, c_void_p]),
     'psi_fit_dp_mode': (c_int, [c_void_p]),
+    'psi_fit_chain_mode': (c_int, [c_void_p]),
     'psi_stream_wait': (c_int, [c_void_p, c_int]),
     'psi_dp_unique_id': (c_int, [c_void_p]),
     'psi_dp_comm_create': (c_int, [c_void_p, c_void_p, c_int, c_int]),
```
